# graphic-goose/ferreus_rbf_rs

Hardware: AMD Instinct MI355X
Metric: BBFMM matvecs/s (higher is better)
Workload: dtype f64; 1 GPU; 10000000 uniform 3D points, LinearRbf, order 7, 1 rhs, adaptive sparse tree, ACA eps=1e-7, set_weights + evaluate at the sources; points=10000000, kernel=LinearRbf, order=7, nrhs=1, parallelism=single GPU

## Files before the change

ferreus_rbf_rs_amd/_lib.py:

```python
from __future__ import annotations

import ctypes
import os

HERE = os.path.dirname(os.path.abspath(__file__))
LIB_PATH = os.environ.get("FERREUS_BBFMM_HIP_LIB") or os.path.join(HERE, "libferreus_bbfmm_hip.so")

OK, POINT_OUTSIDE_TREE, KERNEL_NO_GRADIENTS, BAD_ARGUMENT, DEVICE_ERROR, UNSUPPORTED, CALLBACK_FAILED = range(7)
FLAG_HOST_ONLY = 1
FLAG_M2L_SHARED_BASIS = 2
FLAG_DIRECT_SMALL_W_LEAVES = 4
FLAG_DETERMINISTIC = 8
N_PHASES = 11
PHASE_NAMES = ["gather", "P2M", "M2M", "M2L_stage1", "M2L_stage2", "P2L", "L2L", "P2P", "M2P",
               "L2P", "scatter"]

c_i32, c_i64, c_f64, c_u32 = ctypes.c_int32, ctypes.c_int64, ctypes.c_double, ctypes.c_uint32
c_p = ctypes.c_void_p


class Params(ctypes.Structure):
    _fields_ = [("max_points_per_cell", c_i64), ("compression_type", c_i32),
                ("epsilon", c_f64), ("eval_chunk_size", c_i64)]

# ... 67 lines not shown
    "bbfmm_isosurface_curvature_weight": (ctypes.c_int, [c_p, c_p, c_i32, c_p, c_p, c_p, c_p]),
    "bbfmm_isosurface_curvature_stats": (ctypes.c_int, [c_p, c_i32, c_p]),
    "bbfmm_isosurface_count": (c_i32, [c_p]),
    "bbfmm_isosurface_size": (ctypes.c_int, [c_p, c_i32, c_p, c_p]),
    "bbfmm_isosurface_copy": (ctypes.c_int, [c_p, c_i32, c_p, c_p]),
    "bbfmm_isosurface_error": (ctypes.c_char_p, [c_p]),
    "bbfmm_isosurface_destroy": (None, [c_p]),
    "bbfmm_prepare_target_subset": (ctypes.c_int, [c_p, c_p, c_i64]),
    "bbfmm_fast_matrix_vector_product": (ctypes.c_int, [c_p, c_p, c_i64, c_i64, c_p, c_i64, c_p,
                                                        c_i64, c_f64, c_p]),
    "bbfmm_matvec_device": (ctypes.c_int, [c_p, c_p, c_i64, c_i32, c_p, c_i64, c_i32]),
    "bbfmm_target_subset_create": (ctypes.c_int, [c_p, c_p, c_i64, c_p]),
    "bbfmm_matvec_subset_device": (ctypes.c_int, [c_p, c_i32, c_p, c_p, c_i32]),
    "bbfmm_stream": (c_p, [c_p]),
    "bbfmm_set_partition": (ctypes.c_int, [c_p, c_i32, c_i32]),
    "bbfmm_partition_row_count": (c_i64, [c_p]),
    "bbfmm_partition_rows": (ctypes.c_int, [c_p, c_p]),
    "bbfmm_partition_coarse_count": (c_i64, [c_p]),
    "bbfmm_matvec_partition_upward": (ctypes.c_int, [c_p, c_p, c_i64, c_i32, c_p, c_p]),
    "bbfmm_matvec_partition_finish": (ctypes.c_int, [c_p, c_p, c_p, c_i64, c_i32, c_p]),
    "bbfmm_partition_world": (c_i32, [c_p]),
    "bbfmm_partition_rank": (c_i32, [c_p]),
    "bbfmm_partition_bounds": (ctypes.c_int, [c_p, c_i32, c_p]),
    "bbfmm_matvec_partition_finish_sorted": (ctypes.c_int, [c_p, c_p, c_p, c_i64, c_p]),
    "bbfmm_partition_scatter": (ctypes.c_int, [c_p, c_p, c_i32, c_i32, c_i64, c_i32, c_p, c_i64]),
    "bbfmm_debug_partition_upward_counts": (ctypes.c_int, [c_p, c_p, c_p, c_p]),
    "bbfmm_debug_host_copy_rates": (ctypes.c_int, [c_i64, c_p]),
    "bbfmm_get_tree_stats": (ctypes.c_int, [c_p, c_p]),
    "bbfmm_tree_built_on_device": (ctypes.c_int, [c_p]),
    "bbfmm_last_evaluate_at_sources": (ctypes.c_int, [c_p]),
    "bbfmm_debug_targets_are_sources": (ctypes.c_int, [c_p, c_p, c_i64, c_i64]),
    "bbfmm_debug_rows_of_sources": (ctypes.c_int, [c_p, c_p, c_i64, c_i64, c_p]),
    "bbfmm_get_cells": (ctypes.c_int, [c_p, c_p, c_p]),
    "bbfmm_get_leaf_sources": (ctypes.c_int, [c_p, c_p, c_p]),
    "bbfmm_get_list": (ctypes.c_int, [c_p, ctypes.c_char, c_p, c_p, c_p]),
    "bbfmm_get_m2l_ranks": (ctypes.c_int, [c_p, c_p, c_p]),
    "bbfmm_get_m2l_operator": (ctypes.c_int, [c_p, c_i32, c_i32, c_p]),
    "bbfmm_get_m2l_factors": (ctypes.c_int, [c_p, c_i32, c_i32, c_p, c_p]),
    "bbfmm_get_permutation_tables": (ctypes.c_int, [c_p, c_p, c_p, c_p, c_p, c_p]),
    "bbfmm_points_to_leaves": (ctypes.c_int, [c_p, c_p, c_i64, c_i64, c_p, c_p]),
    "bbfmm_set_profiling": (ctypes.c_int, [c_p, c_i32]),
    "bbfmm_get_phase_ms": (ctypes.c_int, [c_p, c_p, c_p]),
    "bbfmm_reset_phase_ms": (ctypes.c_int, [c_p]),
    "bbfmm_mfma_f64_selftest": (ctypes.c_int, [c_p, c_p, c_p]),
    "bbfmm_fp64_valu_selftest": (ctypes.c_int, [c_p, c_p]),
    "bbfmm_debug_kernel_values": (ctypes.c_int, [c_i32, c_i32, ctypes.c_double, ctypes.c_double, c_p, c_i64, c_p, c_p, c_p]),
    "bbfmm_debug_math": (ctypes.c_int, [c_i32, c_i32, c_p, c_i64, c_p, c_p]),
    "bbfmm_debug_dense_m2m": (ctypes.c_int, [c_p, c_i32, c_p]),
    "bbfmm_debug_apply_m2l_tables_host": (ctypes.c_int, [c_p, c_p, c_p]),
    "bbfmm_debug_m2l_variants": (ctypes.c_int, [c_p, c_p, c_p]),
    "bbfmm_debug_m2l_pairs": (ctypes.c_int, [c_p, c_p, c_i64, c_p, c_p]),
    "bbfmm_debug_m2l_pairs_axes": (ctypes.c_int, [c_p, c_p, c_i64, c_p]),
    "bbfmm_debug_m2l_pairs_stage2": (ctypes.c_int, [c_p, c_p, c_i64, c_p, c_p]),
    "bbfmm_debug_m2l_s2_last_ksplit": (ctypes.c_int, [c_p, c_p]),
    "bbfmm_debug_get_coefficients": (ctypes.c_int, [c_p, ctypes.c_char, c_i32, c_p]),
    "bbfmm_debug_morton_encode": (ctypes.c_uint64, [c_i32, c_p, ctypes.c_uint64]),
    "bbfmm_debug_morton_decode": (None, [c_i32, ctypes.c_uint64, c_p, c_p]),
    "bbfmm_debug_morton_neighbours": (c_i32, [c_i32, ctypes.c_uint64, c_p]),
    "bbfmm_debug_direction_vectors": (c_i32, [c_i32, c_p]),
    "bbfmm_debug_reference_vectors": (ctypes.c_int, [c_p, c_p, c_p]),
    "bbfmm_givens_rotation": (None, [c_f64, c_f64, c_p, c_p, c_p]),
    "bbfmm_fgmres": (ctypes.c_int, [c_i64, c_p, c_p, c_p, c_p, c_p, c_p, c_i32, c_i32, c_i32, c_f64,
                                    c_p, c_p, c_p, c_p, c_p]),
    "bbfmm_schwarz_ddm_solver": (ctypes.c_int, [c_i64, c_p, c_p, c_p, c_p, c_p, c_i32, c_i32, c_f64,
                                                c_p, c_p, c_p, c_p, c_p]),
    "bbfmm_rbf_system_apply": (ctypes.c_int, [c_p, c_p, c_p, c_i64]),
    "bbfmm_ddm_params_defaults": (None, [c_p]),
    "bbfmm_ddm_params_for_points": (None, [c_i64, c_p]),
    "bbfmm_ddm_build": (ctypes.c_int, [c_p, c_i64, c_i32, c_i64, c_p, c_p]),
    "bbfmm_ddm_destroy": (None, [c_p]),
    "bbfmm_ddm_num_levels": (c_i32, [c_p]),
    "bbfmm_ddm_level_size": (c_i64, [c_p, c_i32]),
    "bbfmm_ddm_level_points": (ctypes.c_int, [c_p, c_i32, c_p]),
    "bbfmm_ddm_num_domains": (c_i64, [c_p, c_i32]),
    "bbfmm_ddm_domain_size": (c_i64, [c_p, c_i32, c_i64]),
    "bbfmm_ddm_domain": (ctypes.c_int, [c_p, c_i32, c_i64, c_p, c_p, c_p]),
    "bbfmm_schwarz_create": (ctypes.c_int, [c_p, c_p, c_i64, c_i32, c_i64, c_p, c_p, c_p]),
    "bbfmm_schwarz_create_sharded": (ctypes.c_int, [c_p, c_p, c_i64, c_i32, c_i64, c_p, c_p, c_i32, c_i32, c_p, c_i64, c_p, c_p, c_p]),
    "bbfmm_schwarz_factor_bytes": (c_i64, [c_p]),
    "bbfmm_schwarz_domains_owned": (c_i64, [c_p, c_i32, ctypes.POINTER(c_i64), ctypes.POINTER(c_i64)]),
    "bbfmm_schwarz_destroy": (None, [c_p]),
    "bbfmm_schwarz_basis_size": (c_i64, [c_p]),
    "bbfmm_schwarz_num_levels": (c_i32, [c_p]),
    "bbfmm_schwarz_monomial_matrix": (c_p, [c_p]),
    "bbfmm_debug_evaluate_monomials": (ctypes.c_int, [c_p, c_i64, c_i32, c_i64, c_i32, c_p, c_p, c_p]),
    "bbfmm_schwarz_apply": (ctypes.c_int, [c_p, c_p, c_p, c_i64]),
    "bbfmm_schwarz_level_size": (c_i64, [c_p, c_i32]),
    "bbfmm_schwarz_level_points": (ctypes.c_int, [c_p, c_i32, c_p]),
    "bbfmm_schwarz_debug_level_solve": (ctypes.c_int, [c_p, c_i32, c_p, c_p, c_i64, c_i32]),
    "bbfmm_ddm_debug_level_create": (ctypes.c_int, [c_p, c_i64, c_i32, c_i64, c_i64, c_p, c_p, c_p, c_p, c_i32, c_i32, c_p]),
    "bbfmm_ddm_debug_level_destroy": (None, [c_p]),
    "bbfmm_ddm_debug_level_info": (ctypes.c_int, [c_p, c_p]),
    "bbfmm_ddm_debug_level_layout": (ctypes.c_int, [c_p, c_p, c_p, c_p, c_p, c_p]),
    "bbfmm_ddm_debug_level_assembled": (ctypes.c_int, [c_p, c_p]),
    "bbfmm_ddm_debug_level_factor": (ctypes.c_int, [c_p, c_p]),
    "bbfmm_ddm_debug_level_solve": (ctypes.c_int, [c_p, c_p, c_p, c_i64, c_i32]),
    "bbfmm_schwarz_create_ex": (ctypes.c_int, [c_p, c_p, c_i64, c_i32, c_i64, c_p, c_i64, c_p, c_p, c_p]),
    "bbfmm_schwarz_create_sharded_ex": (ctypes.c_int, [c_p, c_p, c_i64, c_i32, c_i64, c_p, c_i64, c_p, c_p, c_i32, c_i32, c_p, c_i64,
                                                       c_p, c_p, c_p]),
    "bbfmm_ddm_debug_level_create_ex": (ctypes.c_int, [c_p, c_i64, c_i32, c_i64, c_p, c_i64, c_i64, c_p, c_p, c_p, c_p, c_i32, c_i32,
                                                       c_p]),
    "bbfmm_global_trend_transform": (ctypes.c_int, [c_i32, c_p, c_p, c_p, c_p]),
    "bbfmm_duplicate_cutoff_distance": (ctypes.c_int, [c_p, c_f64, c_p]),
    "bbfmm_remove_duplicates": (ctypes.c_int, [c_p, c_i64, c_i32, c_i64, c_f64, c_i32, c_p, c_p, c_p]),
    "bbfmm_debug_interpolant_terms": (ctypes.c_int, [c_i32, c_i32, c_p, c_p, c_i64, c_i64, c_p, c_i64, c_p, c_i64, c_p, c_i64]),
    "bbfmm_evaluate_interpolant": (ctypes.c_int, [c_p, c_i32, c_i32, c_p, c_i64, c_i32, c_i64, c_p, c_i64, c_i64, c_p, c_f64,
# ... 76 lines not shown
```

ferreus_rbf_rs_amd/csrc/capi.cpp:

```cpp
#include <cmath>
#include <cstddef>
#include <cstring>
#include <new>
#include <string>
#include <vector>

#include <algorithm>
#include <chrono>
#include <cstdlib>
#include <memory>

#include "device_group.hpp"
#include "ferreus_bbfmm_hip.h"
#include "fmm_tree.hpp"
#include "interpolant_terms.hpp"
#include "field_program.hpp"
#include "closure_triangulate.hpp"
#include "isosurface.hpp"
#include "isosurface_closure.hpp"
#include "isosurface_curvature.hpp"
#include "isosurface_intersect.hpp"
#include "morton.hpp"

struct bbfmm_handle {
// ... 1920 lines not shown
    if (d < 1 || d > 3 || !out) return -1;
    const int(*dirs)[3];
    const int n = bbfmm::direction_vectors(d, &dirs);
    for (int i = 0; i < n; ++i)
        for (int a = 0; a < d; ++a) out[i * d + a] = dirs[i][a];
    return n;
}
int bbfmm_debug_reference_vectors(const bbfmm_handle *h, int32_t *out, int32_t *n_ref_out) {
    if (!h) return BBFMM_BAD_ARGUMENT;
    const bbfmm::Operators &ops = h->tree.ops();
    if (n_ref_out) *n_ref_out = ops.n_ref;
    if (out) std::copy(ops.ref_vecs.begin(), ops.ref_vecs.end(), out);
    return BBFMM_OK;
}

int bbfmm_debug_m2l_variants(const bbfmm_handle *h, int64_t *n_variants, int64_t *n_cells) {
    if (!h) return BBFMM_BAD_ARGUMENT;
    int64_t nv = 0, nc = 0;
    h->tree.m2l_variant_stats(&nv, &nc);
    if (n_variants) *n_variants = nv;
    if (n_cells) *n_cells = nc;
    return BBFMM_OK;
}

int bbfmm_debug_m2l_pairs(const bbfmm_handle *h, int32_t *out, int64_t cap, int64_t *n_out, int32_t *pairs_on) {
    if (!h || !n_out) return BBFMM_BAD_ARGUMENT;
    std::vector<int32_t> v;
    h->tree.debug_m2l_pairs(&v);
    *n_out = static_cast<int64_t>(v.size());
    if (pairs_on) *pairs_on = h->tree.m2l_pairs() ? 1 : 0;
    if (out) std::copy(v.begin(), v.begin() + std::min<int64_t>(cap, *n_out), out);
    return BBFMM_OK;
}

int bbfmm_debug_m2l_pairs_axes(const bbfmm_handle *h, int32_t *out, int64_t cap, int64_t *n_out) {
    if (!h || !n_out) return BBFMM_BAD_ARGUMENT;
    std::vector<int32_t> v;
    h->tree.debug_m2l_pairs_axes(&v);
    *n_out = static_cast<int64_t>(v.size());
    if (out) std::copy(v.begin(), v.begin() + std::min<int64_t>(cap, *n_out), out);
    return BBFMM_OK;
}

int bbfmm_debug_m2l_pairs_stage2(const bbfmm_handle *h, int32_t *out, int64_t cap, int64_t *n_out, int32_t *pairs_on) {
    if (!h || !n_out) return BBFMM_BAD_ARGUMENT;
    std::vector<int32_t> v;
    h->tree.debug_m2l_pairs_stage2(&v);
    *n_out = static_cast<int64_t>(v.size());
    if (pairs_on) *pairs_on = h->tree.m2l_pairs_stage2() ? 1 : 0;
    if (out) std::copy(v.begin(), v.begin() + std::min<int64_t>(cap, *n_out), out);
    return BBFMM_OK;
}

int bbfmm_debug_m2l_s2_last_ksplit(const bbfmm_handle *h, int32_t *ksplit) {
    if (!h || !ksplit) return BBFMM_BAD_ARGUMENT;
    *ksplit = h->tree.debug_m2l_s2_last_ksplit();
    return BBFMM_OK;
}

int bbfmm_debug_get_coefficients(bbfmm_handle *h, char which, int32_t k, double *out) {
    GUARD(h) return h->tree.debug_get_coefficients(which, k, out);
    END_GUARD(h)
}

}

#include "ddm.hpp"
struct bbfmm_ddm {
    bbfmm::DdmTree tree;
};
extern "C" {
void bbfmm_ddm_params_defaults(bbfmm_ddm_params *out) {
    if (!out) return;
    const bbfmm::DdmParams p;
    out->leaf_threshold = p.leaf_threshold;
    out->overlap_quota = p.overlap_quota;
    out->coarse_ratio = p.coarse_ratio;
    out->coarse_threshold = p.coarse_threshold;
}

void bbfmm_ddm_params_for_points(int64_t n, bbfmm_ddm_params *out) {
    if (!out) return;
    bbfmm_ddm_params_defaults(out);
    out->coarse_threshold = std::max<int64_t>(out->coarse_threshold, n / 470 + 1);
}
int bbfmm_ddm_build(const double *points, int64_t n, int32_t d, int64_t ld, const bbfmm_ddm_params *params,
                    bbfmm_ddm **out) {
    if (!out) return BBFMM_BAD_ARGUMENT;
    *out = nullptr;
    bbfmm::DdmParams p;
    if (params) {
        p.leaf_threshold = params->leaf_threshold;
        p.overlap_quota = params->overlap_quota;
        p.coarse_ratio = params->coarse_ratio;
        p.coarse_threshold = params->coarse_threshold;
    }
    bbfmm_ddm *t = new (std::nothrow) bbfmm_ddm();
    if (!t) return BBFMM_DEVICE_ERROR;
    int rc = BBFMM_BAD_ARGUMENT;
    try {
        rc = bbfmm::build_ddm_tree(points, n, d, ld, p, &t->tree);
    } catch (...) {
        rc = BBFMM_DEVICE_ERROR;
    }
    if (rc != BBFMM_OK) {
        delete t;
// ... 43 lines not shown
```

ferreus_rbf_rs_amd/csrc/device.hpp:

```cpp
#pragma once
#include <hip/hip_runtime.h>

#include <cstdint>

#include "kernels.hpp"

namespace bbfmm {

constexpr int kMaxOrder = 16;
constexpr int kM2lTile = 128;
constexpr int kM2lS1Block = 176;
constexpr int kM2lS1BlockPairs = 160;
constexpr int kM2lSlotWindow = 128;
constexpr int kM2lBlkTwoDst = 1 << 30;

struct DevCheb {
    int p, d, n, n_pad;
    double polyn[kMaxOrder * kMaxOrder];
    double nodes[kMaxOrder];
    double xfer[2 * kMaxOrder * kMaxOrder];
};

struct ChebRef {
    const DevCheb *dev;
    int p, d, n, n_pad;
};

struct M2lClass {
    const double *vt_all;
    const int32_t *row_dst;
    const int32_t *row_dst2;
    const int32_t *blk_t0;
    int32_t yb0;
    int32_t n_rows;
    int32_t r_pad16;
    int32_t n_t;
    const double *u_all;
    int32_t k_pad;
    int32_t kp;
    const int32_t *cells;
    int32_t n_cells;
    const int32_t *cslot;
    const int64_t *cbase;
};

struct M2lTileDesc {
    int32_t level_class;
    int32_t first;
    int32_t count;
    int32_t q_first;
    int32_t q_count;
    int32_t pad;
};

void launch_gather_weights(const double *w, int64_t ldw, int K, const int32_t *order, int64_t N,
                           double *w_sorted, hipStream_t s);
void launch_gather_weights_subset(const double *w, int64_t ldw, int K, const int32_t *order, const int32_t *pos, int64_t n_pos,
                                  int64_t N, double *w_sorted, hipStream_t s);
constexpr int kMaxScatterParts = 64;
struct ScatterParts {
    int n;
    int64_t bound[kMaxScatterParts + 1];
};
void launch_scatter_parts(const double *all, const ScatterParts &parts, int64_t m_max, int K, const int32_t *order, double *out,
                          int64_t ldo, hipStream_t s);
void launch_sum_slots(const double *slots, int n_slots, int64_t len, double *out, hipStream_t s);
void launch_scatter_output(const double *out_sorted, int64_t n, int K, const int32_t *perm,
                           double *out, int64_t ldo, int accumulate, hipStream_t s);
void launch_gather_rows(const double *src, int64_t ld_src, int ncols, const int32_t *idx, int64_t n,
                        double *dst, int64_t ld_dst, hipStream_t s);

void launch_p2m(const ChebRef &ch, const double *const *src_xyz, const double *w_sorted, int64_t N,
                int K, int64_t C, const int32_t *leaf_cells, int n_leaves, const int32_t *pt_begin,
                const int32_t *pt_end, const double *centers, const double *lengths, double *M,
                hipStream_t s);
int launch_m2m(const ChebRef &ch, int K, int64_t C, const int32_t *parents, int n_parents,
               const int64_t *child_ptr, const int32_t *child_idx, const int32_t *octant, double *M,
               hipStream_t s);
int launch_l2l(const ChebRef &ch, int K, int64_t C, const int32_t *cells, int n_cells,
               const int32_t *parent, const int32_t *octant, const uint8_t *active, double *L,
               hipStream_t s);

void launch_m2l_stage1(const M2lClass *classes, const M2lTileDesc *tiles, const int32_t *tile_idx, int n_tiles,
                       int n_pad, int max_slot_t, int K, int64_t C, const double *M, double *cbuf,
                       int64_t cbuf_len, hipStream_t s, bool own_blocks = false, int max_blocks = 8, int ne16 = 0, int s_ee = 0,
                       int s_eo = 0);
void launch_m2l_parity(const double *M, int n_pad, double *Mp, int n_par, int ne16, int n_e, int n_o, int p, int64_t rows,
                       hipStream_t s);
struct M2lParityOffsets {
    int32_t v[4];
};
void launch_m2l_parity2(const double *M, int n_pad, double *Mp, int n_par, M2lParityOffsets off, int p, int p2, int64_t rows,
                        hipStream_t s);
void launch_m2l_stage2(const M2lClass *classes, const M2lTileDesc *tiles, const int32_t *tile_idx, int n_tiles,
                       int n_pad, int K, int64_t C, const double *cbuf, int64_t cbuf_len,
                       const uint16_t *qlist, double *L, hipStream_t s, bool allow_ksplit = true);
struct M2lS2PairsPlan {
    int ga, gb, ce, co;
    int ne16() const { return 16 * ga * ce; }
    int n_par() const { return 16 * (ga * ce + gb * co); }
};
M2lS2PairsPlan m2l_s2_pairs_plan(int groups_even, int groups_odd);
bool launch_m2l_stage2_pairs(const M2lClass *classes, const M2lTileDesc *tiles, const int32_t *tile_idx, int n_tiles,
                             const M2lS2PairsPlan &plan, int K, int64_t C, const double *cbuf, int64_t cbuf_len,
                             const uint16_t *qlist, double *Lp, hipStream_t s, bool allow_ksplit = true, int *ksplit_out = nullptr);
void launch_m2l_unparity(const double *Lp, int n_par, int ne16, double *L, int n, int n_pad, int n_e, int n_o, int p, int64_t rows,
                         hipStream_t s);
void launch_m2l_zero_segments(const int32_t *segs, int64_t n_segs, int K, double *cbuf, int64_t cbuf_len, hipStream_t s);
void launch_m2l_basis(const M2lClass *classes, const M2lTileDesc *tiles, int n_tiles, int in_ld, int out_ld, int K,
                      int64_t C, const double *in, double *out, hipStream_t s);
void launch_small_gemm(bool trans_a, int M, int N, int Kd, const double *A, int64_t lda, const double *B, int64_t ldb,
                       double *Cm, int64_t ldc, hipStream_t s);

struct M2lAssembleTv {
    int32_t perm;
    int32_t rank;
    int32_t row;
    int64_t vt_off;
    int64_t u_off;
};
struct M2lAssembleClass {
    const M2lAssembleTv *src, *tgt;
    int32_t n_src, n_tgt, r_pad16, k_pad, max_rank;
    int32_t n_e, n_o, ne16, n_par, p;
    int32_t u_npar, u_ne16, u_rows, u_ne, u_no;
    int32_t s1_axes;
    M2lParityOffsets s1_off;
};
void launch_m2l_assemble(const M2lAssembleClass &c, int n, int n_pad, bool compressed, const double *ops,
                         const int32_t *invperm, double *vt_all, double *u_all, hipStream_t s);

struct DirectJobs {
    int n_jobs;
    const int32_t *job_cell;
    const int32_t *tgt_begin, *tgt_end;
    const int64_t *run_ptr;
    const int32_t *runs;
};
void launch_p2p(const KernelSpec &ks, int d, const DirectJobs &jobs, const double *const *tgt_xyz,
                int64_t n_tgt, const double *const *src_xyz, const double *w_sorted, int64_t N, int K,
                double *out_sorted, double *grad_sorted, hipStream_t s, bool fixed_plan = false);
constexpr int kSymMaxRhs = 4;
void launch_p2p_sym(const KernelSpec &ks, int n_jobs, const int32_t *tgt_begin, const int32_t *tgt_end,
                    const int64_t *run_range, int n_leaf_jobs, const int32_t *l_tgt_begin, const int32_t *l_tgt_end,
                    const int64_t *l_run_range, int n_wave_jobs, const int32_t *w_tgt_begin, const int32_t *w_tgt_end,
                    const int64_t *w_run_range, const int32_t *runs3, int32_t tgt_off, const double *const *src_xyz,
                    const double *w_sorted, int64_t ldw, int K, double *out_sorted, int64_t ldo, hipStream_t s);
int p2p_sym_rows_per_job();
int p2p_sym3_rows_per_job();
int p2p_sym_wave_rows();
int64_t p2p_sym_wave_min_jobs();
int wx_sym_rows_per_job();
int wx_sym3_rows_per_job();
void launch_wx_sym(const KernelSpec &ks, const ChebRef &ch, int n_jobs, const int32_t *tgt_begin, const int32_t *tgt_end,
                   const int64_t *w_range, int n_leaf_jobs, const int32_t *l_tgt_begin, const int32_t *l_tgt_end,
                   const int64_t *l_w_range, const int32_t *w_cells, const double *centers, const double *lengths,
                   const double *const *src_xyz, const double *w_sorted, int64_t ldw, int K, const double *M, double *L,
                   int64_t ld_ml, double *out_sorted, int64_t ldo, int out_off, int out_n, hipStream_t s);
void launch_m2p(const KernelSpec &ks, const ChebRef &ch, int n_jobs, const int32_t *tgt_begin,
                const int32_t *tgt_end, const int64_t *w_begin, const int64_t *w_end,
                const int32_t *w_cells,
                const double *centers, const double *lengths, const double *const *tgt_xyz,
                int64_t n_tgt, int K, int64_t C, const double *M, double *out_sorted,
                double *grad_sorted, hipStream_t s, bool fixed_plan = false);
void launch_p2l(const KernelSpec &ks, const ChebRef &ch, int n_jobs, const int32_t *cells,
                const int64_t *run_ptr, const int32_t *runs, const double *centers,
                const double *lengths, const double *const *src_xyz, const double *w_sorted,
                int64_t N, int K, int64_t C, double *L, hipStream_t s);
void launch_l2p(const ChebRef &ch, int n_jobs, const int32_t *leaf_cells, const int32_t *tgt_begin,
                const int32_t *tgt_end, const double *centers, const double *lengths,
                const double *const *tgt_xyz, int64_t n_tgt, int K, int64_t C, const double *L,
                double *out_sorted, double *grad_sorted, hipStream_t s);

bool l2p_order_supported(int p, int d);

int mfma_f64_selftest(double *tflops, int *layout_errors, double *info);
int valu_f64_selftest(double *tflops, double *mhz);
int debug_kernel_values_device(const KernelSpec &ks, const double *r2, int64_t n, double *value, double *value_g, double *factor);
int debug_math_device(int which, const double *x, int64_t n, double *out, double *out2);

// ... 2 lines not shown
```

ferreus_rbf_rs_amd/csrc/device_m2l.hip:

```cpp
#include "device_common.hpp"

#include <cmath>

namespace bbfmm {

typedef __attribute__((address_space(3))) void *lptr_t;

__device__ inline unsigned lds_offset(const double *p) {
    return static_cast<unsigned>(reinterpret_cast<uintptr_t>((lptr_t)p));
}
__device__ inline unsigned uniform_u32(unsigned v) { return __builtin_amdgcn_readfirstlane(v); }
__device__ inline const double *uniform_ptr(const double *p) {
    const uintptr_t v = reinterpret_cast<uintptr_t>(p);
    const unsigned lo = __builtin_amdgcn_readfirstlane(static_cast<unsigned>(v));
    const unsigned hi = __builtin_amdgcn_readfirstlane(static_cast<unsigned>(v >> 32));
    return reinterpret_cast<const double *>((static_cast<uintptr_t>(hi) << 32) | lo);
}
__device__ inline void dma16(const double *g, unsigned lds_wave_byte_offset) {
    asm volatile("s_mov_b32 m0, %1\n\ts_nop 0\n\tglobal_load_lds_dwordx4 %0, off" ::"v"(g),
                 "s"(uniform_u32(lds_wave_byte_offset))
                 : "memory");
}
__device__ inline void dma4(const int32_t *g, unsigned lds_wave_byte_offset) {
    asm volatile("s_mov_b32 m0, %1\n\ts_nop 0\n\tglobal_load_lds_dword %0, off" ::"v"(g),
// ... 392 lines not shown
    const int zmax = n_tiles * 8 < n_cu ? std::max(8, std::min(max_blocks, 32)) : 8;
    int zsplit = 1;
    double best = 1e300;
    for (int z = 1; z <= zmax; ++z) {
        const double rounds = std::ceil(static_cast<double>(n_tiles) * z / n_cu);
        const double cost = rounds / z * (1.0 + 0.005 * z);
        if (cost < best - 1e-12) {
            best = cost;
            zsplit = z;
        }
    }
    const int n_colblocks = own_blocks ? 1 : zsplit;
    if (ne16 > 0) {
        const int64_t packed = static_cast<int64_t>(ne16) | (static_cast<int64_t>(s_ee & 0xffff) << 32) | (static_cast<int64_t>(s_eo & 0x7fff) << 48);
        m2l_gemm_launch<kM2lS1BlockPairs / 16, 1, 1, true>(classes, tiles, n_tiles, n_pad, 0, n_colblocks, K, C, M, packed, cbuf, cbuf_len,
                                                      nullptr, slot_t, tile_idx, s);
        return;
    }
    m2l_dispatch_chunks<1>(kM2lS1Block / 16, classes, tiles, n_tiles, n_pad, n_colblocks, K, C, M, 0, cbuf, cbuf_len, nullptr,
                           slot_t, tile_idx, s);
}

static int m2l_s2_ksplit(int64_t wgs, bool allow_ksplit) {
    static const int ks_env = [] {
        const int v = env_int("BBFMM_M2L_S2_KSPLIT", 0);
        return v >= 1 && v <= 32 ? v : 0;
    }();
    if (!allow_ksplit) return 1;
    if (ks_env > 0) return ks_env;
    const int n_cu = device_cu_count();
    int ksplit = 1;
    if (wgs * 2 <= static_cast<int64_t>(kM2lS2KsplitFill) * n_cu) {
        double best = 1e300;
        for (int ks = 1; ks <= 16; ++ks) {
            const double cost = std::ceil(static_cast<double>(wgs * ks) / n_cu) * (0.05 + 1.0 / ks);
            if (cost < best - 1e-12) {
                best = cost;
                ksplit = ks;
            }
        }
    }
    return ksplit;
}

void launch_m2l_stage2(const M2lClass *classes, const M2lTileDesc *tiles, const int32_t *tile_idx, int n_tiles,
                       int n_pad, int K, int64_t C, const double *cbuf, int64_t cbuf_len, const uint16_t *qlist,
                       double *L, hipStream_t s, bool allow_ksplit) {
    if (n_tiles == 0) return;
    static const int z = env_int("BBFMM_M2L_S2_ZSPLIT", 2) == 1 ? 1 : 2;
    const int ksplit = m2l_s2_ksplit(static_cast<int64_t>(n_tiles) * z * K, allow_ksplit);
    m2l_dispatch_chunks<2>(n_pad / 16, classes, tiles, n_tiles, n_pad, z, K, C, cbuf, cbuf_len, L, 0, qlist, ksplit > 1 ? ksplit : 0, tile_idx, s);
}

template <int NG16>
__device__ __forceinline__ void m2l_s2_pairs_body(const M2lClass &cls, const M2lTileDesc &tile, int n_par, int g16, bool odd,
                                                  int zk, int ksplit, int64_t C, const double *__restrict__ in, int64_t in_len,
                                                  double *__restrict__ out, const uint16_t *__restrict__ qlist,
                                                  const int32_t *__restrict__ tile_idx, double *lds) {
    const int kr = blockIdx.y;
    const int tid = threadIdx.x, wave = tid >> 6, lane = tid & 63;
    const int ld = n_par;
    const int q_lo = tile.q_count * zk / ksplit;
    const int nq = tile.q_count * (zk + 1) / ksplit - q_lo;
    const uint16_t *ql = qlist + tile.q_first + q_lo;
    const int kp = cls.kp, kp16 = kp >> 4;
    const double *opbase = cls.u_all + 16 * g16;

    constexpr int OP_CHUNKS = 2 * NG16;
    constexpr int NCH = (OP_CHUNKS + 7) / 8;
    constexpr int OP_DOUBLES = OP_CHUNKS * 128;
    constexpr int BUF = OP_DOUBLES + 4096;
    constexpr int NP = NG16 / 2, NS = NG16 & 1;
    unsigned voff[NCH];
#pragma unroll
    for (int i = 0; i < NCH; ++i) {
        const int c = wave + 8 * i;
        if (c < 4 * NP) {
            const int e = c / (NP > 0 ? NP : 1), pr = c - e * NP, k = lane >> 4, p = lane & 15;
            voff[i] = (unsigned)(((4 * k + e) * ld + 32 * pr + 2 * p) * 8);
        } else {
            const int e = 2 * (c - 4 * NP) + (lane >> 5), r = lane & 31, k = r >> 3, pair = r & 7;
            voff[i] = (unsigned)(((4 * k + e) * ld + 32 * NP + 2 * pair) * 8);
        }
    }
    auto cell_p = [&](int pos) {
        const int q = pos < tile.count ? pos : 0;
        return tile.pad ? tile_idx[tile.first + q] : tile.first + q;
    };
    const double *cptr[2];
#pragma unroll
    for (int h = 0; h < 2; ++h) {
        const int tg = 2 * h + (lane >> 5), eh = (lane >> 4) & 1, k = (lane >> 2) & 3, j = lane & 3;
        const int p = cell_p(wave * 16 + 4 * tg + j);
        cptr[h] = in + (int64_t)kr * in_len + cls.cbase[p] + 4 * k + 2 * eh;
    }
    const unsigned lds0 = lds_offset(lds);
    const int64_t qstride = (int64_t)16 * ld;
    auto stage = [&](int qi, int buf) {
        const int q = (int)uniform_u32(ql[qi]);
#pragma unroll
        for (int i = 0; i < NCH; ++i)
            if (wave + 8 * i < OP_CHUNKS)
                dma16s(opbase + q * qstride, voff[i], lds0 + (unsigned)(buf * BUF + (wave + 8 * i) * 128) * 8u);
#pragma unroll
        for (int h = 0; h < 2; ++h)
            dma16(cptr[h] + kp + 16 * q, lds0 + (unsigned)(buf * BUF + OP_DOUBLES + 2048 + (2 * wave + h) * 128) * 8u);
        if (q < kp16) {
#pragma unroll
            for (int h = 0; h < 2; ++h)
                dma16(cptr[h] + 16 * q, lds0 + (unsigned)(buf * BUF + OP_DOUBLES + (2 * wave + h) * 128) * 8u);
        }
        return q < kp16;
    };

    double acc[4][NG16];
#pragma unroll
    for (int tg = 0; tg < 4; ++tg)
#pragma unroll
        for (int g = 0; g < NG16; ++g) acc[tg][g] = 0.0;

    const int bk = lane >> 4, bj = lane & 3;
    const bool wave_live = wave * 16 < tile.count;
    const int di = lane >> 4, db = (lane >> 2) & 3, dj = lane & 3;
    const double sgn = odd ? -1.0 : 1.0;
    bool pair_cur = false;
    if (nq > 0) pair_cur = stage(0, 0);
    wait_dma_and_barrier();
    for (int sidx = 0; sidx < nq; ++sidx) {
        const double *op = lds + (sidx & 1) * BUF + lane;
        const double2 *op2 = reinterpret_cast<const double2 *>(lds + (sidx & 1) * BUF) + lane;
        const double *cx = lds + (sidx & 1) * BUF + OP_DOUBLES + wave * 256 + (bk * 4 + bj) * 2;
        bool pair_next = false;
        if (sidx + 1 < nq) pair_next = stage(sidx + 1, (sidx + 1) & 1);
        if (wave_live) {
            double bq[4][4];
#pragma unroll
            for (int tg = 0; tg < 4; ++tg)
#pragma unroll
                for (int eh = 0; eh < 2; ++eh) {
                    const double2 y = *reinterpret_cast<const double2 *>(cx + 2048 + ((tg * 2 + eh) * 16) * 2);
                    bq[tg][2 * eh] = y.x;
                    bq[tg][2 * eh + 1] = y.y;
                }
            if (pair_cur) {
#pragma unroll
                for (int tg = 0; tg < 4; ++tg)
#pragma unroll
                    for (int eh = 0; eh < 2; ++eh) {
                        const double2 x = *reinterpret_cast<const double2 *>(cx + ((tg * 2 + eh) * 16) * 2);
                        bq[tg][2 * eh] = x.x + sgn * bq[tg][2 * eh];
                        bq[tg][2 * eh + 1] = x.y + sgn * bq[tg][2 * eh + 1];
                    }
            }
#pragma unroll
            for (int e = 0; e < 4; ++e) {
#pragma unroll
                for (int pr = 0; pr < NP; ++pr) {
                    const double2 a = op2[(e * NP + pr) * 64];
#pragma unroll
                    for (int tg = 0; tg < 4; ++tg) {
                        acc[tg][2 * pr] = __builtin_amdgcn_mfma_f64_4x4x4f64(a.x, bq[tg][e], acc[tg][2 * pr], 0, 0, 0);
                        acc[tg][2 * pr + 1] = __builtin_amdgcn_mfma_f64_4x4x4f64(a.y, bq[tg][e], acc[tg][2 * pr + 1], 0, 0, 0);
                    }
                }
                if (NS) {
                    const double a = op[4 * NP * 128 + e * 64];
#pragma unroll
                    for (int tg = 0; tg < 4; ++tg)
                        acc[tg][NG16 - 1] = __builtin_amdgcn_mfma_f64_4x4x4f64(a, bq[tg][e], acc[tg][NG16 - 1], 0, 0, 0);
                }
            }
        }
        pair_cur = pair_next;
        wait_dma_and_barrier();
    }
    const int col0 = 16 * g16;
#pragma unroll
    for (int tg = 0; tg < 4; ++tg) {
        const int tp = wave * 16 + 4 * tg + dj;
        if (tp < tile.count) {
            const int cell = cls.cells[cell_p(tp)];
            double *Lc = out + ((int64_t)kr * C + cell) * n_par + col0;
            if (ksplit > 1) {
#pragma unroll
                for (int pr = 0; pr < NP; ++pr) {
                    unsafeAtomicAdd(Lc + 32 * pr + 2 * (4 * db + di), acc[tg][2 * pr]);
                    unsafeAtomicAdd(Lc + 32 * pr + 2 * (4 * db + di) + 1, acc[tg][2 * pr + 1]);
                }
                if (NS) unsafeAtomicAdd(Lc + 32 * NP + 4 * db + di, acc[tg][NG16 - 1]);
            } else {
#pragma unroll
                for (int pr = 0; pr < NP; ++pr)
                    *reinterpret_cast<double2 *>(Lc + 32 * pr + 2 * (4 * db + di)) = make_double2(acc[tg][2 * pr], acc[tg][2 * pr + 1]);
                if (NS) Lc[32 * NP + 4 * db + di] = acc[tg][NG16 - 1];
            }
        }
    }
}

template <int GA, int GB>
__global__ __launch_bounds__(512, 1) void m2l_s2_pairs_kernel(const M2lClass *__restrict__ classes, const M2lTileDesc *__restrict__ tiles,
                                                              int n_par, int ce, int co, int ksplit, int64_t C,
                                                              const double *__restrict__ in, int64_t in_len, double *__restrict__ out,
                                                              const uint16_t *__restrict__ qlist, const int32_t *__restrict__ tile_idx) {
    extern __shared__ double lds[];
    const M2lTileDesc tile = tiles[blockIdx.x];
    const M2lClass cls = classes[tile.level_class];
    const int zcols = ce + co;
    const int zk = (int)blockIdx.z / zcols, zc = (int)blockIdx.z - zk * zcols;
    if (zc < ce) m2l_s2_pairs_body<GA>(cls, tile, n_par, zc * GA, false, zk, ksplit, C, in, in_len, out, qlist, tile_idx, lds);
    else m2l_s2_pairs_body<GB>(cls, tile, n_par, ce * GA + (zc - ce) * GB, true, zk, ksplit, C, in, in_len, out, qlist, tile_idx, lds);
}

#define M2L_S2_PAIR_WIDTHS(X) X(13, 10) X(13, 11) X(8, 8) X(7, 7) X(5, 4) X(4, 4) X(2, 2) X(1, 1)
#define M2L_S2_WIDTH_ENTRY(A, B) {A, B},
static constexpr int kM2lS2PairWidths[][2] = {M2L_S2_PAIR_WIDTHS(M2L_S2_WIDTH_ENTRY)};
#undef M2L_S2_WIDTH_ENTRY

M2lS2PairsPlan m2l_s2_pairs_plan(int groups_even, int groups_odd) {
    M2lS2PairsPlan best{1, 1, std::max(groups_even, 1), std::max(groups_odd, 1)};
    int best_cost = 1 << 30;
    for (const auto &w : kM2lS2PairWidths) {
        const int ce = std::max(1, (groups_even + w[0] - 1) / w[0]), co = std::max(1, (groups_odd + w[1] - 1) / w[1]);
        const int cost = ce * (w[0] + 2) + co * (w[1] + 2);
        if (cost < best_cost) {
            best_cost = cost;
            best = M2lS2PairsPlan{w[0], w[1], ce, co};
        }
    }
    return best;
}

template <int GA, int GB>
static void m2l_s2_pairs_launch(const M2lClass *classes, const M2lTileDesc *tiles, const int32_t *tile_idx, int n_tiles,
                                const M2lS2PairsPlan &plan, int ksplit, int K, int64_t C, const double *cbuf, int64_t cbuf_len,
                                const uint16_t *qlist, double *Lp, hipStream_t s) {
    const size_t lds = 2 * sizeof(double) * (size_t)(2 * (GA > GB ? GA : GB) * 128 + 4096);
    static std::atomic<uint64_t> attr_set[4] = {{0}, {0}, {0}, {0}};
    (void)allow_large_dynamic_lds(reinterpret_cast<const void *>(&m2l_s2_pairs_kernel<GA, GB>), lds, attr_set);
    hipLaunchKernelGGL((m2l_s2_pairs_kernel<GA, GB>), dim3(n_tiles, K, (plan.ce + plan.co) * ksplit), dim3(512), lds, s, classes, tiles,
                       plan.n_par(), plan.ce, plan.co, ksplit, C, cbuf, cbuf_len, Lp, qlist, tile_idx);
}

bool launch_m2l_stage2_pairs(const M2lClass *classes, const M2lTileDesc *tiles, const int32_t *tile_idx, int n_tiles,
                             const M2lS2PairsPlan &plan, int K, int64_t C, const double *cbuf, int64_t cbuf_len,
                             const uint16_t *qlist, double *Lp, hipStream_t s, bool allow_ksplit, int *ksplit_out) {
    if (n_tiles == 0) return true;
    const int ksplit = m2l_s2_ksplit(static_cast<int64_t>(n_tiles) * (plan.ce + plan.co) * K, allow_ksplit);
    if (ksplit_out) *ksplit_out = ksplit;
#define M2L_S2_DISPATCH(A, B)                                                                                            \
    if (plan.ga == A && plan.gb == B) {                                                                                  \
        m2l_s2_pairs_launch<A, B>(classes, tiles, tile_idx, n_tiles, plan, ksplit, K, C, cbuf, cbuf_len, qlist, Lp, s);  \
        return true;                                                                                                     \
    }
    M2L_S2_PAIR_WIDTHS(M2L_S2_DISPATCH)
#undef M2L_S2_DISPATCH
    return false;
}

__global__ __launch_bounds__(256) void m2l_unparity_kernel(const double *__restrict__ Lp, int n_par, int ne16, double *__restrict__ L,
                                                           int n, int n_pad, int n_e, int n_o, int p, int p1, int64_t rows) {
    const int64_t row = static_cast<int64_t>(blockIdx.x) * 4 + (threadIdx.x >> 6);
    if (row >= rows) return;
    const double *src = Lp + row * n_par;
    double *dst = L + row * n_pad;
    for (int j = threadIdx.x & 63; j < n_e; j += 64) {
        const double e = src[j];
        if (j < n_o) {
            const double o = src[ne16 + j];
            dst[j] = e + o;
            dst[j + (p - 1 - 2 * (j / p1)) * p1] = e - o;
        } else {
            dst[j] = e;
        }
    }
    for (int j = n + (threadIdx.x & 63); j < n_pad; j += 64) dst[j] = 0.0;
}

void launch_m2l_unparity(const double *Lp, int n_par, int ne16, double *L, int n, int n_pad, int n_e, int n_o, int p, int64_t rows,
                         hipStream_t s) {
    if (rows <= 0) return;
    const int p1 = n_e / ((p + 1) / 2);
    hipLaunchKernelGGL(m2l_unparity_kernel, dim3(static_cast<unsigned>((rows + 3) / 4)), dim3(256), 0, s, Lp, n_par, ne16, L, n, n_pad, n_e,
                       n_o, p, p1, rows);
}

__global__ __launch_bounds__(256) void m2l_parity_kernel(const double *__restrict__ M, int n_pad, double *__restrict__ Mp, int n_par,
                                                         int ne16, int n_e, int n_o, int p, int p1, int64_t rows) {
    const int64_t row = static_cast<int64_t>(blockIdx.x) * 4 + (threadIdx.x >> 6);
    if (row >= rows) return;
    const double *src = M + row * n_pad;
    double *dst = Mp + row * n_par;
    for (int j = threadIdx.x & 63; j < n_e; j += 64) {
        const double v = src[j];
        if (j < n_o) {
            const double w = src[j + (p - 1 - 2 * (j / p1)) * p1];
            dst[j] = v + w;
            dst[ne16 + j] = v - w;
        } else {
            dst[j] = v;
        }
    }
}

void launch_m2l_parity(const double *M, int n_pad, double *Mp, int n_par, int ne16, int n_e, int n_o, int p, int64_t rows,
                       hipStream_t s) {
    if (rows <= 0) return;
    const int p1 = n_e / ((p + 1) / 2);
    hipLaunchKernelGGL(m2l_parity_kernel, dim3(static_cast<unsigned>((rows + 3) / 4)), dim3(256), 0, s, M, n_pad, Mp, n_par, ne16, n_e,
                       n_o, p, p1, rows);
}

__global__ __launch_bounds__(256) void m2l_parity2_kernel(const double *__restrict__ M, int n_pad, double *__restrict__ Mp, int n_par,
                                                          M2lParityOffsets off, int p, int p2, int64_t rows) {
    const int64_t row = static_cast<int64_t>(blockIdx.x) * 4 + (threadIdx.x >> 6);
    if (row >= rows) return;
    const double *src = M + row * n_pad;
    double *dst = Mp + row * n_par;
    const int h = (p + 1) / 2, f = p / 2;
    for (int e = threadIdx.x & 63; e < h * h * p2; e += 64) {
        const int i0 = e / (h * p2), i1 = (e - i0 * h * p2) / p2, r = e - (i0 * h + i1) * p2;
        const int m = (i0 * p + i1) * p2 + r;
        const int dx = (p - 1 - 2 * i0) * p * p2, dy = (p - 1 - 2 * i1) * p2;
        const bool cx = i0 >= f, cy = i1 >= f;
        const double v = src[m], vx = src[m + dx], vy = src[m + dy], vxy = src[m + dx + dy];
        const double e0 = cx ? v : v + vx, e1 = cx ? vy : vy + vxy, o0 = v - vx, o1 = vy - vxy;
        const int je = (i0 * h + i1) * p2 + r, jo = (i0 * f + i1) * p2 + r;
        dst[off.v[0] + je] = cy ? e0 : e0 + e1;
        if (!cy) dst[off.v[1] + jo] = e0 - e1;
        if (!cx) dst[off.v[2] + je] = cy ? o0 : o0 + o1;
        if (!cx && !cy) dst[off.v[3] + jo] = o0 - o1;
    }
}

void launch_m2l_parity2(const double *M, int n_pad, double *Mp, int n_par, M2lParityOffsets off, int p, int p2, int64_t rows,
                        hipStream_t s) {
    if (rows <= 0) return;
// ... 127 lines not shown
    const bool cx = i0 >= f, cy = i1 >= f;
    const int32_t *inv = invperm + static_cast<int64_t>(tv.perm) * n;
    const double *s0 = ops + tv.vt_off + static_cast<int64_t>(inv[m]) * tv.rank;
    const double *sx = ops + tv.vt_off + static_cast<int64_t>(inv[m + dx]) * tv.rank;
    const double *sy = ops + tv.vt_off + static_cast<int64_t>(inv[m + dy]) * tv.rank;
    const double *sxy = ops + tv.vt_off + static_cast<int64_t>(inv[m + dx + dy]) * tv.rank;
    const int je = (i0 * h + i1) * p2 + r, jo = (i0 * f + i1) * p2 + r;
    double *dee = vt_all + static_cast<int64_t>(c.s1_off.v[0] + je) * c.r_pad16 + tv.row;
    double *deo = vt_all + static_cast<int64_t>(c.s1_off.v[1] + jo) * c.r_pad16 + tv.row;
    double *doe = vt_all + static_cast<int64_t>(c.s1_off.v[2] + je) * c.r_pad16 + tv.row;
    double *doo = vt_all + static_cast<int64_t>(c.s1_off.v[3] + jo) * c.r_pad16 + tv.row;
    const double wx = cx ? 1.0 : 0.5, wy = cy ? 1.0 : 0.5;
    for (int kk = 0; kk < tv.rank; ++kk) {
        const double v = s0[kk], vx = sx[kk], vy = sy[kk], vxy = sxy[kk];
        const double e0 = cx ? v : v + vx, e1 = cx ? vy : vy + vxy, o0 = v - vx, o1 = vy - vxy;
        dee[kk] = wx * wy * (cy ? e0 : e0 + e1);
        if (!cy) deo[kk] = wx * wy * (e0 - e1);
        if (!cx) doe[kk] = wx * wy * (cy ? o0 : o0 + o1);
        if (!cx && !cy) doo[kk] = wx * wy * (o0 - o1);
    }
}

__global__ __launch_bounds__(256) void assemble_u_kernel(M2lAssembleClass c, int n, int n_pad, const double *__restrict__ ops,
                                                         const int32_t *__restrict__ invperm, double *__restrict__ u_all) {
    const int pos = blockIdx.y;
    const M2lAssembleTv tv = c.tgt[pos];
    const int64_t t = static_cast<int64_t>(blockIdx.x) * 256 + threadIdx.x;
    if (t >= static_cast<int64_t>(tv.rank) * n) return;
    const int kk = static_cast<int>(t / n), i = static_cast<int>(t % n);
    u_all[static_cast<int64_t>(tv.row + kk) * n_pad + i] = ops[tv.u_off + static_cast<int64_t>(kk) * n + invperm[static_cast<int64_t>(tv.perm) * n + i]];
}

__global__ __launch_bounds__(256) void assemble_u_parity_kernel(M2lAssembleClass c, int n, const double *__restrict__ ops,
                                                                const int32_t *__restrict__ invperm, double *__restrict__ u_all) {
    const M2lAssembleTv tv = c.tgt[blockIdx.y];
    const int64_t t = static_cast<int64_t>(blockIdx.x) * 256 + threadIdx.x;
    if (t >= static_cast<int64_t>(tv.rank) * c.u_ne) return;
    const int kk = static_cast<int>(t / c.u_ne), i = static_cast<int>(t % c.u_ne);
    const int p1 = n / c.p;
    const int ri = i + (c.p - 1 - 2 * (i / p1)) * p1;
    const int32_t *inv = invperm + static_cast<int64_t>(tv.perm) * n;
    const double *ucol = ops + tv.u_off + static_cast<int64_t>(kk) * n;
    double *dst = u_all + static_cast<int64_t>(tv.row + kk) * c.u_npar;
    const double a = ucol[inv[i]];
    if (i >= c.u_no) {
        dst[i] = a;
    } else {
        const double b = ucol[inv[ri]];
        dst[i] = 0.5 * (a + b);
        dst[c.u_ne16 + i] = 0.5 * (a - b);
    }
}

void launch_m2l_assemble(const M2lAssembleClass &c, int n, int n_pad, bool compressed, const double *ops,
                         const int32_t *invperm, double *vt_all, double *u_all, hipStream_t s) {
    (void)hipMemsetAsync(vt_all, 0, static_cast<size_t>(c.n_e > 0 ? c.n_par : n_pad) * c.r_pad16 * sizeof(double), s);
    (void)hipMemsetAsync(u_all, 0, (c.u_npar > 0 ? static_cast<size_t>(c.u_rows) * c.u_npar : static_cast<size_t>(c.k_pad) * n_pad) * sizeof(double), s);
    if (c.n_src > 0 && c.n_e > 0 && c.s1_axes == 2) {
        const int h = (c.p + 1) / 2, n_ee = h * h * (n / (c.p * c.p));
        hipLaunchKernelGGL(assemble_vt_parity2_kernel, dim3(static_cast<unsigned>((static_cast<int64_t>(c.n_src) * n_ee + 255) / 256)), dim3(256),
                           0, s, c, n, ops, invperm, vt_all);
    } else if (c.n_src > 0 && c.n_e > 0)
        hipLaunchKernelGGL(assemble_vt_parity_kernel, dim3(static_cast<unsigned>((static_cast<int64_t>(c.n_src) * c.n_e + 255) / 256)), dim3(256),
                           0, s, c, n, ops, invperm, vt_all);
    else if (c.n_src > 0)
        hipLaunchKernelGGL(assemble_vt_kernel, dim3(static_cast<unsigned>((static_cast<int64_t>(c.n_src) * n + 255) / 256)), dim3(256), 0, s, c, n, n_pad,
                           compressed ? 1 : 0, ops, invperm, vt_all);
    if (c.n_tgt > 0 && c.max_rank > 0 && c.u_npar > 0)
        hipLaunchKernelGGL(assemble_u_parity_kernel, dim3(static_cast<unsigned>((static_cast<int64_t>(c.max_rank) * c.u_ne + 255) / 256), c.n_tgt),
                           dim3(256), 0, s, c, n, ops, invperm, u_all);
    else if (c.n_tgt > 0 && c.max_rank > 0)
        hipLaunchKernelGGL(assemble_u_kernel, dim3(static_cast<unsigned>((static_cast<int64_t>(c.max_rank) * n + 255) / 256), c.n_tgt), dim3(256), 0, s, c,
                           n, n_pad, ops, invperm, u_all);
}

}
```

ferreus_rbf_rs_amd/csrc/fmm_m2l_tables.cpp:

```cpp
#include "fmm_tree_impl.hpp"

namespace bbfmm {

void FmmTree::fill_m2l_operator_arrays(const HostM2lClass &hc, std::vector<double> *vt_all,
                                       std::vector<double> *u_all) const {
    const int n_pad = round_up(ops_.n, 32);
    vt_all->resize(static_cast<size_t>(m2l_pairs_ ? m2l_npar_ : n_pad) * hc.r_pad16);
    u_all->resize(m2l_pairs2_ ? static_cast<size_t>(hc.k_pad - hc.kp) * m2l_s2_plan_.n_par() : static_cast<size_t>(hc.k_pad) * n_pad);
    fill_m2l_operator_arrays(hc, vt_all->data(), u_all->data());
}

void FmmTree::fill_m2l_operator_arrays(const HostM2lClass &hc, double *vt_all, double *u_all) const {
    const int n = ops_.n, n_pad = round_up(n, 32);
    const bool compressed = ops_.compression != kCompressionNone;
    const auto &lops = ops_.m2l[hc.level];
    auto zero = [](double *p, size_t len) {
        parallel_for_chunks(static_cast<int64_t>(len), int64_t(1) << 18, [&](int64_t b, int64_t e) {
            std::memset(p + b, 0, static_cast<size_t>(e - b) * sizeof(double));
        });
    };
    zero(vt_all, static_cast<size_t>(m2l_pairs_ ? m2l_npar_ : n_pad) * hc.r_pad16);
    zero(u_all, m2l_pairs2_ ? static_cast<size_t>(hc.k_pad - hc.kp) * m2l_s2_plan_.n_par() : static_cast<size_t>(hc.k_pad) * n_pad);
    struct RowSrc {
        const M2lOperator *op;
// ... 21 lines not shown
                for (int kk = 0; kk < r; ++kk) {
                    double v = 0.0;
                    for (int g = 0; g < 4; ++g)
                        if (nd[g] >= 0) v += sg[g] * rs.op->vt[static_cast<size_t>(rs.inv[nd[g]]) * r + kk];
                    dst[rs.first_row + kk] = w * v;
                }
            }
        });
    } else if (m2l_pairs_) {
        parallel_for(m2l_ne_, 8, [&](int64_t j) {
            const bool centre = j >= m2l_no_;
            const int rj = m2l_rho(static_cast<int>(j));
            double *de = vt_all + static_cast<size_t>(j) * hc.r_pad16;
            double *dod = vt_all + static_cast<size_t>(m2l_ne16_ + j) * hc.r_pad16;
            for (const RowSrc &rs : row_src) {
                const int r = rs.op->rank;
                const double *s0 = &rs.op->vt[static_cast<size_t>(rs.inv[j]) * r], *s1 = &rs.op->vt[static_cast<size_t>(rs.inv[rj]) * r];
                for (int kk = 0; kk < r; ++kk) {
                    if (centre) {
                        de[rs.first_row + kk] = s0[kk];
                    } else {
                        de[rs.first_row + kk] = 0.5 * (s0[kk] + s1[kk]);
                        dod[rs.first_row + kk] = 0.5 * (s0[kk] - s1[kk]);
                    }
                }
            }
        });
    } else {
        parallel_for(n, 8, [&](int64_t m) {
            double *dst = vt_all + static_cast<size_t>(m) * hc.r_pad16;
            for (const RowSrc &rs : row_src) {
                const int r = rs.op->rank;
                const int im = rs.inv[m];
                if (compressed) {
                    const double *src = &rs.op->vt[static_cast<size_t>(im) * r];
                    for (int kk = 0; kk < r; ++kk) dst[rs.first_row + kk] = src[kk];
                } else {
                    dst[rs.first_row + im] = 1.0;
                }
            }
        });
    }
    if (m2l_pairs2_) {
        const int n_par = m2l_s2_plan_.n_par(), ne16 = m2l_s2_plan_.ne16();
        parallel_for(static_cast<int64_t>(hc.tgt_tv.size()), 1, [&](int64_t pos) {
            if (hc.tgt_pair[pos] == -2) return;
            const int tv = hc.tgt_tv[pos];
            const M2lOperator &op = lops[ops_.ref_lookup[tv]];
            const int32_t *inv = &ops_.invperm[static_cast<size_t>(ops_.perm_lookup[tv]) * n];
            const int row0 = hc.tgt_off[pos] - (hc.tgt_pair[pos] >= 0 ? 0 : hc.kp);
            for (int kk = 0; kk < op.rank; ++kk) {
                double *dst = u_all + static_cast<size_t>(row0 + kk) * n_par;
                const double *ucol = &op.u[static_cast<size_t>(kk) * n];
                for (int i = 0; i < m2l_ne_; ++i) {
                    const double a = ucol[inv[i]], b = ucol[inv[m2l_rho(i)]];
                    if (i >= m2l_no_) {
                        dst[i] = a;
                    } else {
                        dst[i] = 0.5 * (a + b);
                        dst[ne16 + i] = 0.5 * (a - b);
                    }
                }
            }
        });
        return;
    }
    parallel_for(static_cast<int64_t>(hc.tgt_tv.size()), 1, [&](int64_t pos) {
        const int tv = hc.tgt_tv[pos];
        const M2lOperator &op = lops[ops_.ref_lookup[tv]];
        const int32_t *inv = &ops_.invperm[static_cast<size_t>(ops_.perm_lookup[tv]) * n];
        for (int kk = 0; kk < op.rank; ++kk) {
            double *dst = u_all + static_cast<size_t>(hc.tgt_off[pos] + kk) * n_pad;
            const double *ucol = &op.u[static_cast<size_t>(kk) * n];
            for (int i = 0; i < n; ++i) dst[i] = ucol[inv[i]];
        }
    });
}

int FmmTree::build_m2l_tables() {
    const HostTree &t = tree_;
    const int d = d_, n = ops_.n;
    const int ncls = 1 << d, nvec = ops_.n_vec;
    const bool compressed = ops_.compression != kCompressionNone;
    m2l_host_.clear();
    m2l_variants_.clear();
    m2l_tiles1_h_.clear();
    m2l_tile_idx1_h_.clear();
    m2l_classes_h_.clear();
    m2l_tiles_h_.clear();
    m2l_qlist_h_.clear();
    m2l_batches_.clear();
    m2l_batch_of_class_.clear();
    m2l_group_ops_.clear();
    cbuf_batch_len_ = 0;
    cbuf_total_len_ = 0;
    m2l_flops_k1_ = 0;
    m2l_flops_level_.clear();
    if (t.depth < 2) return BBFMM_OK;
    if (!host_only_) {
        size_t free_b = 0, total_b = 0;
        if (hipMemGetInfo(&free_b, &total_b) == hipSuccess && total_b > 0)
            m2l_budget_bytes_ = std::max<int64_t>(int64_t(4) << 30, static_cast<int64_t>(total_b / 16));
    }
    if (const char *e = std::getenv("BBFMM_M2L_CBUF_MB")) {
        const double mb = std::atof(e);
        if (mb > 0) m2l_budget_bytes_ = static_cast<int64_t>(mb * 1048576.0);
    }

    auto comp = [&](int tv, int a) { return ops_.all_vecs[static_cast<size_t>(tv) * d + a]; };
    {
        const char *e = std::getenv("BBFMM_M2L_S1_PAIRS");
        m2l_pairs_ = !(e && std::atoi(e) == 0) && compressed && !shared_basis_ && d >= 2 && ops_.p >= 2;
        const char *e2 = std::getenv("BBFMM_M2L_S2_PAIRS");
        m2l_pairs2_ = !(e2 && std::atoi(e2) == 0) && compressed && !shared_basis_ && d >= 2 && ops_.p >= 2;
        m2l_partner_.assign(static_cast<size_t>(nvec), -1);
        m2l_s1_block_ = m2l_pairs_ ? kM2lS1BlockPairs : kM2lS1Block;
        const int p1 = n / ops_.p;
        m2l_ne_ = (ops_.p + 1) / 2 * p1;
        m2l_no_ = ops_.p / 2 * p1;
        m2l_ne16_ = round_up(m2l_ne_, 16);
        m2l_npar_ = m2l_ne16_ + round_up(m2l_no_, 16);
        m2l_s2_plan_ = m2l_s2_pairs_plan(m2l_ne16_ / 16, round_up(m2l_no_, 16) / 16);
        for (int tv = 0; tv < nvec && (m2l_pairs_ || m2l_pairs2_); ++tv) {
            if (comp(tv, 0) == 0) continue;
            int rt = -1;
            for (int u = 0; u < nvec && rt < 0; ++u) {
                bool same = comp(u, 0) == -comp(tv, 0);
                for (int a = 1; a < d; ++a) same = same && comp(u, a) == comp(tv, a);
                if (same) rt = u;
            }
            if (rt < 0 || ops_.ref_lookup[rt] != ops_.ref_lookup[tv]) continue;
            const int32_t *it = &ops_.invperm[static_cast<size_t>(ops_.perm_lookup[tv]) * n];
            const int32_t *ir = &ops_.invperm[static_cast<size_t>(ops_.perm_lookup[rt]) * n];
            bool ok = true;
            for (int m = 0; m < n && ok; ++m) ok = ir[m] == it[m2l_rho(m)];
            if (ok) m2l_partner_[static_cast<size_t>(tv)] = rt;
        }
        m2l_partner_y_.assign(static_cast<size_t>(nvec), -1);
        for (int tv = 0; tv < nvec && m2l_pairs_; ++tv) {
            if (comp(tv, 1) == 0) continue;
            int rt = -1;
            for (int u = 0; u < nvec && rt < 0; ++u) {
                bool same = comp(u, 1) == -comp(tv, 1);
                for (int a = 0; a < d; ++a) same = same && (a == 1 || comp(u, a) == comp(tv, a));
                if (same) rt = u;
            }
            if (rt < 0 || ops_.ref_lookup[rt] != ops_.ref_lookup[tv]) continue;
            const int32_t *it = &ops_.invperm[static_cast<size_t>(ops_.perm_lookup[tv]) * n];
            const int32_t *ir = &ops_.invperm[static_cast<size_t>(ops_.perm_lookup[rt]) * n];
            bool ok = true;
            for (int m = 0; m < n && ok; ++m) ok = ir[m] == it[m2l_rho_y(m)];
            if (ok) m2l_partner_y_[static_cast<size_t>(tv)] = rt;
        }
    }
    auto far = [&](int tv) {
        int mx = 0;
        for (int a = 0; a < d; ++a) mx = std::max(mx, std::abs(comp(tv, a)));
        return mx >= 2;
    };
    std::vector<std::vector<int>> tgt_list(ncls), src_list(ncls), tpos_tgt(ncls, std::vector<int>(nvec, -1)),
        tpos_src(ncls, std::vector<int>(nvec, -1));
    for (int o = 0; o < ncls; ++o)
        for (int tv = 0; tv < nvec; ++tv) {
            if (!far(tv)) continue;
            bool okt = true, oks = true;
            for (int a = 0; a < d; ++a) {
                const int oa = (o >> a) & 1, ta = comp(tv, a);
                okt = okt && ta >= oa - 3 && ta <= oa + 2;
                oks = oks && ta >= -2 - oa && ta <= 3 - oa;
            }
            if (okt) {
                tpos_tgt[o][tv] = static_cast<int>(tgt_list[o].size());
                tgt_list[o].push_back(tv);
            }
            if (oks) {
                tpos_src[o][tv] = static_cast<int>(src_list[o].size());
                src_list[o].push_back(tv);
            }
        }
    auto pairs_first = [&](std::vector<int> *list, std::vector<int> *tpos) {
        std::vector<int> ordered, singles;
        std::vector<uint8_t> used(static_cast<size_t>(nvec), 0);
        for (int tv : *list) {
            const int rt = m2l_partner_[static_cast<size_t>(tv)];
            if (used[static_cast<size_t>(tv)]) continue;
            if (rt >= 0 && (*tpos)[rt] >= 0 && m2l_partner_[static_cast<size_t>(rt)] == tv) {
                const int first = comp(tv, 0) > 0 ? tv : rt;
                ordered.push_back(first);
                ordered.push_back(first == tv ? rt : tv);
                used[static_cast<size_t>(tv)] = used[static_cast<size_t>(rt)] = 1;
            } else {
                singles.push_back(tv);
// ... 97 lines not shown
        for (int i = 1; i < 4; ++i) off2.v[i] = off2.v[i - 1] + round_up(len[i - 1], 16);
        const int npar2 = off2.v[3] + round_up(len[3], 16);
        std::vector<std::vector<int>> src_xy = src_list;
        for (int o = 0; o < ncls; ++o) order_axes(&src_xy[o], nullptr);
        for (int level = 2; level <= t.depth; ++level) {
            std::vector<uint8_t> has(static_cast<size_t>(ncls), 0);
            for (int64_t c = t.level_ptr[level]; c < t.level_ptr[level + 1]; ++c) has[t.octant[c]] = 1;
            for (int o = 0; o < ncls; ++o) {
                if (!has[static_cast<size_t>(o)]) continue;
                std::vector<int32_t> marks;
                const int rows1 = mark_pairs_at(level, 1, src_list[o], &marks, nullptr, nullptr, nullptr, nullptr);
                const int rows2 = mark_pairs_at(level, 2, src_xy[o], &marks, nullptr, nullptr, nullptr, nullptr);
                m2l_work_[0] += static_cast<int64_t>(round_up(std::max(rows1, 1), m2l_s1_block_) / m2l_s1_block_) * (m2l_npar_ / 16);
                m2l_work_[1] += static_cast<int64_t>(round_up(std::max(rows2, 1), m2l_s1_block_) / m2l_s1_block_) * (npar2 / 16);
            }
        }
        const char *e = std::getenv("BBFMM_M2L_S1_AXES");
        const int want = e ? std::atoi(e) : 0;
        if (want == 2 || (want != 1 && m2l_work_[1] < m2l_work_[0])) {
            m2l_axes_ = 2;
            m2l_s1_off_ = off2;
            m2l_ne16_ = off2.v[2];
            m2l_npar_ = npar2;
            m2l_s_ee_ = off2.v[1] / 16;
            m2l_s_eo_ = (off2.v[2] - off2.v[1]) / 16;
            for (int o = 0; o < ncls; ++o) {
                src_list[o] = src_xy[o];
                for (size_t i = 0; i < src_list[o].size(); ++i) tpos_src[o][src_list[o][i]] = static_cast<int>(i);
            }
            m2l_par_node_.assign(static_cast<size_t>(npar2) * 4, -1);
            m2l_par_sign_.assign(static_cast<size_t>(npar2) * 4, 0);
            for (int i0 = 0; i0 < h; ++i0)
                for (int i1 = 0; i1 < h; ++i1)
                    for (int r = 0; r < p2; ++r) {
                        const int m = (i0 * p + i1) * p2 + r;
                        const bool cx = i0 >= f, cy = i1 >= f;
                        const int nodes[4] = {m, m2l_rho(m), m2l_rho_y(m), m2l_rho_y(m2l_rho(m))};
                        const int je = (i0 * h + i1) * p2 + r, jo = (i0 * f + i1) * p2 + r;
                        for (int part = 0; part < 4; ++part) {
                            const bool ox = part >= 2, oy = part & 1;
                            if ((ox && cx) || (oy && cy)) continue;
                            const size_t k = static_cast<size_t>(off2.v[part] + (oy ? jo : je));
                            for (int g = 0; g < 4; ++g) {
                                const bool gx = g & 1, gy = g & 2;
                                if ((gx && cx) || (gy && cy)) continue;
                                m2l_par_node_[4 * k + g] = nodes[g];
                                m2l_par_sign_[4 * k + g] = static_cast<int8_t>(((gx && ox) != (gy && oy)) ? -1 : 1);
                            }
                        }
                    }
        }
    }
    std::vector<std::vector<int32_t>> tgt_pair(ncls);
    for (int o = 0; o < ncls; ++o) {
        const std::vector<int> &tl = tgt_list[o];
        tgt_pair[o].assign(tl.size(), -1);
        for (size_t pos = 0; m2l_pairs2_ && pos + 1 < tl.size(); ++pos)
            if (m2l_partner_[static_cast<size_t>(tl[pos])] == tl[pos + 1] && m2l_partner_[static_cast<size_t>(tl[pos + 1])] == tl[pos]) {
                tgt_pair[o][pos] = static_cast<int32_t>(pos + 1);
                tgt_pair[o][pos + 1] = -2;
                ++pos;
            }
    }
    auto target_class = [&](int o, int tv) {
        int oc = 0;
        for (int a = 0; a < d; ++a) {
            const int v = ((o >> a) & 1) + comp(tv, a);
            oc |= (((v % 2) + 2) % 2) << a;
        }
        return oc;
    };

    std::vector<int32_t> pos_in_class(t.n_cells(), -1);
    int64_t bad_pairs = 0;
    auto slot_layout = [&](int level, std::vector<std::vector<int>> *off_tgt, std::vector<int> *k_pad, std::vector<int> *kp_out = nullptr) {
        const auto &lops = ops_.m2l[level];
        off_tgt->assign(ncls, {});
        k_pad->assign(ncls, 0);
        if (kp_out) kp_out->assign(ncls, 0);
        for (int o = 0; o < ncls; ++o) {
            int lead = 0;
            for (size_t pos = 0; pos < tgt_list[o].size(); ++pos)
                if (tgt_pair[o][pos] >= 0) lead += round_up(lops[ops_.ref_lookup[tgt_list[o][pos]]].rank, 2);
            const int kp = round_up(lead, 16);
            int off = 0, off_s = 2 * kp;
            for (size_t pos = 0; pos < tgt_list[o].size(); ++pos) {
                const int seg = round_up(lops[ops_.ref_lookup[tgt_list[o][pos]]].rank, 2);
                if (tgt_pair[o][pos] >= 0) {
                    (*off_tgt)[o].push_back(off);
                } else if (tgt_pair[o][pos] == -2) {
                    (*off_tgt)[o].push_back(kp + off);
                    off += seg;
                } else {
                    (*off_tgt)[o].push_back(off_s);
                    off_s += seg;
                }
            }
            (*k_pad)[o] = round_up(std::max(off_s, 16), 16);
            if (kp_out) (*kp_out)[o] = kp;
        }
    };
    std::vector<int> level_groups(static_cast<size_t>(t.depth) + 1, 1);
    std::vector<std::vector<int>> batch_of(static_cast<size_t>(t.depth) + 1, std::vector<int>(ncls, -1));
    {
        const int64_t budget = std::max<int64_t>(m2l_budget_bytes_ / 8 - 128, 1);
        std::vector<std::vector<int64_t>> class_len(static_cast<size_t>(t.depth) + 1, std::vector<int64_t>(ncls, 0));
        for (int level = 2; level <= t.depth; ++level) {
            std::vector<std::vector<int>> off_tgt;
            std::vector<int> k_pad;
            slot_layout(level, &off_tgt, &k_pad);
            for (int64_t c = t.level_ptr[level]; c < t.level_ptr[level + 1]; ++c) class_len[level][t.octant[c]] += k_pad[t.octant[c]];
        }
        int64_t cur_len = 0;
        for (int level = 2; level <= t.depth; ++level) {
            int64_t len = 0;
            for (int64_t v : class_len[level]) len += v;
            cbuf_total_len_ += len;
            int G = 1;
            if (len > budget)
                for (G = 2; G < ncls; G *= 2) {
                    int64_t worst = 0;
                    for (int g = 0; g < G; ++g) {
                        int64_t gl = 0;
                        for (int o = g * ncls / G; o < (g + 1) * ncls / G; ++o) gl += class_len[level][o];
                        worst = std::max(worst, gl);
                    }
                    if (worst <= budget) break;
                }
            if (G >= ncls) {
                G = ncls;
                int64_t worst = 0;
                for (int64_t v : class_len[level]) worst = std::max(worst, v);
                if (worst > budget && std::getenv("BBFMM_VERBOSE"))
                    std::fprintf(stderr, "[bbfmm] warning: level %d needs %.1f MB of M2L intermediate per right-hand side even "
                                         "with one batch per target class; the budget of %.1f MB (BBFMM_M2L_CBUF_MB) is exceeded\n",
                                 level, worst * 8.0 / 1048576.0, m2l_budget_bytes_ / 1048576.0);
            }
            level_groups[level] = G;
            if (G == 1 && !m2l_batches_.empty() && m2l_batches_.back().groups == 1 && cur_len + len <= budget) {
                m2l_batches_.back().level_hi = level;
                cur_len += len;
                for (int o = 0; o < ncls; ++o) batch_of[level][o] = static_cast<int>(m2l_batches_.size()) - 1;
                continue;
            }
            for (int g = 0; g < G; ++g) {
                M2lBatch b;
                b.level_lo = b.level_hi = level;
                b.groups = G;
                b.group = g;
                for (int o = g * ncls / G; o < (g + 1) * ncls / G; ++o) batch_of[level][o] = static_cast<int>(m2l_batches_.size());
                m2l_batches_.push_back(b);
            }
            cur_len = len;
        }
    }
    std::vector<std::vector<M2lTileDesc>> tiles1_of_batch(m2l_batches_.size());
    std::vector<int32_t> variant_batch;
    std::vector<std::vector<int32_t>> zero_of_batch(m2l_batches_.size());
    for (int level = 2; level <= t.depth; ++level) {
        const auto &lops = ops_.m2l[level];
        auto rank_of = [&](int tv) { return lops[ops_.ref_lookup[tv]].rank; };
        std::vector<std::vector<int>> off_tgt;
        std::vector<int> k_pad, kp_cls;
        slot_layout(level, &off_tgt, &k_pad, &kp_cls);
        const size_t first_class = m2l_host_.size();
        auto mark_pairs = [&](const std::vector<int> &tvs, std::vector<int32_t> *src_pair) {
            return mark_pairs_at(level, m2l_axes_, tvs, src_pair, nullptr, nullptr, nullptr, nullptr);
        };
        auto stage1_rows = [&](int o, const std::vector<int> &tvs, HostM2lClass *hcp) {
            HostM2lClass &hc = *hcp;
            hc.n_t = static_cast<int>(tvs.size());
            std::vector<int32_t> first_row;
            hc.n_rows = mark_pairs_at(level, m2l_axes_, tvs, &hc.src_pair, &first_row, &hc.src_kind, &hc.yb0, &hc.pad_cols);
            hc.r_pad16 = round_up(std::max(hc.n_rows, 1), m2l_s1_block_);
            if (hc.yb0 < 0) hc.yb0 = hc.r_pad16 / m2l_s1_block_;
            hc.row_tpos.assign(hc.r_pad16, -1);
            hc.row_off.assign(hc.r_pad16, 0);
            hc.row_tpos2.assign(hc.r_pad16, -1);
            hc.row_off2.assign(hc.r_pad16, 0);
            hc.src_tv = tvs;
            int row = 0;
            hc.src_row0.assign(tvs.size(), 0);
            hc.src_row1.assign(tvs.size(), 0);
            for (size_t pos = 0; pos < tvs.size(); ++pos) {
                if (hc.src_pair[pos] == -2) {
                    hc.src_row0[pos] = hc.src_row0[pos - 1];
                    hc.src_row1[pos] = hc.src_row1[pos - 1];
                    continue;
                }
                const int tv = tvs[pos];
                const int oc = target_class(o, tv);
                const int base_off = off_tgt[oc][tpos_tgt[oc][tv]];
                int base_off2 = 0;
                if (hc.src_pair[pos] >= 0) {
                    const int tv2 = tvs[pos + 1], oc2 = target_class(o, tv2);
                    base_off2 = off_tgt[oc2][tpos_tgt[oc2][tv2]];
                }
                if (rank_of(tv) > 0) row = first_row[pos];
                hc.src_row0[pos] = row;
                for (int kk = 0; kk < rank_of(tv); ++kk, ++row) {
                    hc.row_tpos[row] = static_cast<int32_t>(pos);
                    hc.row_off[row] = base_off + kk;
                    if (hc.src_pair[pos] >= 0) {
                        hc.row_tpos2[row] = static_cast<int32_t>(pos + 1);
                        hc.row_off2[row] = base_off2 + kk;
                    }
                }
                hc.src_row1[pos] = row;
                row = round_up(row, 2);
            }
            const int n_blk = hc.r_pad16 / m2l_s1_block_;
            m2l_max_blocks_ = std::max(m2l_max_blocks_, n_blk);
            hc.blk_t0.assign(n_blk, 0);
            hc.row_dst.assign(hc.r_pad16, -1);
            hc.row_dst2.assign(hc.r_pad16, -1);
            for (int b = 0; b < n_blk; ++b) {
                int t0 = -1, t1 = -1;
                bool two = false;
                for (int r = b * m2l_s1_block_; r < (b + 1) * m2l_s1_block_; ++r) {
                    if (hc.row_tpos[r] < 0) continue;
                    if (t0 < 0) t0 = hc.row_tpos[r];
                    t1 = std::max(hc.row_tpos[r], hc.row_tpos2[r]);
                    two = two || hc.row_tpos2[r] >= 0;
                }
                if (t0 < 0) continue;
                hc.blk_t0[b] = t0 | (two ? kM2lBlkTwoDst : 0);
                m2l_slot_t_ = std::max(m2l_slot_t_, t1 - t0 + 1);
                for (int r = b * m2l_s1_block_; r < (b + 1) * m2l_s1_block_; ++r) {
                    if (hc.row_tpos[r] < 0) continue;
                    if (hc.row_off[r] >= (1 << 24) || hc.row_off2[r] >= (1 << 24)) return false;
                    hc.row_dst[r] = ((hc.row_tpos[r] - t0) << 24) | hc.row_off[r];
                    if (hc.row_tpos2[r] >= 0) hc.row_dst2[r] = ((hc.row_tpos2[r] - t0) << 24) | hc.row_off2[r];
                }
            }
            return true;
        };
        m2l_host_.resize(first_class + ncls);
        m2l_group_ops_.resize(first_class + ncls);
        for (int64_t c = t.level_ptr[level]; c < t.level_ptr[level + 1]; ++c)
            m2l_host_[first_class + t.octant[c]].cells.push_back(static_cast<int32_t>(c));
        {
            std::vector<uint64_t> key(static_cast<size_t>(t.level_ptr[level + 1] - t.level_ptr[level]));
            const int64_t c_lo = t.level_ptr[level];
            for (int64_t c = c_lo; c < t.level_ptr[level + 1]; ++c) {
                uint64_t hsh = 1469598103934665603ull;
                const int64_t nv = t.v.ptr[c + 1] - t.v.ptr[c];
                uint64_t bits[6] = {0, 0, 0, 0, 0, 0};
                for (int64_t q = t.v.ptr[c]; q < t.v.ptr[c + 1]; ++q) {
                    const int tv = t.v_tidx[q];
                    if (tv >= 0 && tv < 384) bits[tv >> 6] |= 1ull << (tv & 63);
                }
                for (uint64_t b : bits) hsh = (hsh ^ b) * 1099511628211ull;
                key[static_cast<size_t>(c - c_lo)] = (static_cast<uint64_t>(1023 - std::min<int64_t>(nv, 1023)) << 54) | (hsh >> 10);
            }
            parallel_for(ncls, 1, [&](int64_t o) {
                auto &cells = m2l_host_[first_class + static_cast<size_t>(o)].cells;
                std::stable_sort(cells.begin(), cells.end(), [&](int32_t a, int32_t b) {
                    return key[static_cast<size_t>(a - c_lo)] < key[static_cast<size_t>(b - c_lo)];
                });
                for (size_t i = 0; i < cells.size(); ++i) pos_in_class[cells[i]] = static_cast<int32_t>(i);
            });
        }
        for (int o = 0; o < ncls; ++o) {
            HostM2lClass &hc = m2l_host_[first_class + o];
            hc.level = level;
            hc.octant = o;
            hc.n_t = static_cast<int>(src_list[o].size());
            hc.k_pad = k_pad[o];
            hc.kp = kp_cls[o];
            hc.tgt_pair = tgt_pair[o];
            if (!stage1_rows(o, src_list[o], &hc)) return fail(BBFMM_BAD_ARGUMENT, "M2L slot too long for the packed row table");
            if (hc.cells.empty()) continue;
            hc.tgt_tv = tgt_list[o];
            hc.tgt_off = off_tgt[o];
            if (host_only_) fill_m2l_operator_arrays(hc, &hc.vt_all, &hc.u_all);
            hc.cbase.resize(hc.cells.size());
            int64_t &cursor = m2l_batches_[static_cast<size_t>(batch_of[level][o])].len;
            for (size_t i = 0; i < hc.cells.size(); ++i) {
                hc.cbase[i] = cursor;
                cursor += hc.k_pad;
            }
            hc.cslot.resize(hc.cells.size() * static_cast<size_t>(hc.n_t));
            {
                int32_t *cs = hc.cslot.data();
                parallel_for_chunks(static_cast<int64_t>(hc.cslot.size()), int64_t(1) << 18, [&](int64_t b, int64_t e) {
                    std::fill(cs + b, cs + e, int32_t(-1));
                });
            }
        }
        {
            const int64_t b0 = t.level_ptr[level], nb_cells = t.level_ptr[level + 1] - b0;
            constexpr int64_t kChunkB = 2048;
            const int64_t nch = (nb_cells + kChunkB - 1) / kChunkB;
            std::vector<double> flops_part(static_cast<size_t>(std::max<int64_t>(nch, 1)), 0.0);
            std::vector<int64_t> bad_part(static_cast<size_t>(std::max<int64_t>(nch, 1)), 0);
            parallel_for_chunks(nb_cells, kChunkB, [&](int64_t lo, int64_t hi) {
                double fl = 0.0;
                int64_t bad = 0;
                for (int64_t B = b0 + lo; B < b0 + hi; ++B) {
                    const HostM2lClass &hb = m2l_host_[first_class + t.octant[B]];
                    const int64_t base = hb.cbase[pos_in_class[B]];
                    for (int64_t q = t.v.ptr[B]; q < t.v.ptr[B + 1]; ++q) {
                        const int32_t V = t.v.idx[q];
                        const int tv = t.v_tidx[q];
                        HostM2lClass &hv = m2l_host_[first_class + t.octant[V]];
                        const int ps = (tv >= 0 && tv < nvec) ? tpos_src[t.octant[V]][tv] : -1;
                        if (ps < 0 || t.level[V] != level || tpos_tgt[t.octant[B]][tv] < 0) {
                            ++bad;
                            continue;
                        }
                        hv.cslot[static_cast<size_t>(pos_in_class[V]) * hv.n_t + ps] = static_cast<int32_t>(base / 2);
                        const int r = rank_of(tv);
                        fl += compressed ? 4.0 * n * r : 2.0 * n * static_cast<double>(n);
                    }
                }
                flops_part[static_cast<size_t>(lo / kChunkB)] = fl;
                bad_part[static_cast<size_t>(lo / kChunkB)] = bad;
            });
            double level_flops = 0.0;
            for (double f : flops_part) level_flops += f;
            m2l_flops_k1_ += level_flops;
            if (m2l_flops_level_.size() <= static_cast<size_t>(level)) m2l_flops_level_.resize(static_cast<size_t>(level) + 1, 0.0);
            m2l_flops_level_[static_cast<size_t>(level)] = level_flops;
// ... 521 lines not shown
                          cbuf.begin() + 2 * (static_cast<int64_t>(m2l_zero_h_[static_cast<size_t>(2 * z)]) + m2l_zero_h_[static_cast<size_t>(2 * z + 1)]), 0.0);
        for (int32_t ti = mb.t1_first; ti < mb.t1_first + mb.t1_count; ++ti) {
            const M2lTileDesc &td = m2l_tiles1_h_[static_cast<size_t>(ti)];
            const bool variant = static_cast<size_t>(td.level_class) >= m2l_host_.size();
            const HostM2lClass &hc = variant ? m2l_variants_[static_cast<size_t>(td.level_class) - m2l_host_.size()]
                                             : m2l_host_[static_cast<size_t>(td.level_class)];
            if (hc.vt_all.empty()) return BBFMM_UNSUPPORTED;
            if (m2l_batch_of_class_[static_cast<size_t>(td.level_class)] != static_cast<int32_t>(b)) return BBFMM_BAD_ARGUMENT;
            for (int32_t q = 0; q < td.count; ++q) {
                const size_t pos = static_cast<size_t>(td.pad ? m2l_tile_idx1_h_[static_cast<size_t>(td.first + q)] : td.first + q);
                ++seen[hc.cells[pos]];
                const double *Mv = M + static_cast<size_t>(hc.cells[pos]) * n;
                for (int row = 0; row < hc.n_rows; ++row) {
                    if (hc.row_tpos[row] < 0) continue;
                    const int32_t slot = hc.cslot[pos * hc.n_t + hc.row_tpos[row]];
                    if (m2l_pairs_) {
                        const int32_t slot2 = hc.row_tpos2[row] >= 0 ? hc.cslot[pos * hc.n_t + hc.row_tpos2[row]] : -1;
                        if (slot < 0 && slot2 < 0) continue;
                        const double *mp = &Mp[static_cast<size_t>(hc.cells[pos]) * m2l_npar_];
                        double a = 0.0, bsum = 0.0;
                        if (row / m2l_s1_block_ >= hc.yb0) {
                            for (int j = 0; j < m2l_npar_; ++j) {
                                const bool y_odd = (j >= m2l_s1_off_.v[1] && j < m2l_s1_off_.v[2]) || j >= m2l_s1_off_.v[3];
                                (y_odd ? bsum : a) += hc.vt_all[static_cast<size_t>(j) * hc.r_pad16 + row] * mp[j];
                            }
                        } else {
                            for (int j = 0; j < m2l_ne16_; ++j) a += hc.vt_all[static_cast<size_t>(j) * hc.r_pad16 + row] * mp[j];
                            for (int j = m2l_ne16_; j < m2l_npar_; ++j) bsum += hc.vt_all[static_cast<size_t>(j) * hc.r_pad16 + row] * mp[j];
                        }
                        if (slot >= 0) cbuf[static_cast<size_t>(slot) * 2 + hc.row_off[row]] = a + bsum;
                        if (slot2 >= 0) cbuf[static_cast<size_t>(slot2) * 2 + hc.row_off2[row]] = a - bsum;
                        continue;
                    }
                    if (slot < 0) continue;
                    double s = 0.0;
                    for (int m = 0; m < n; ++m) s += hc.vt_all[static_cast<size_t>(m) * hc.r_pad16 + row] * Mv[m];
                    cbuf[static_cast<size_t>(slot) * 2 + hc.row_off[row]] = s;
                }
            }
        }
        for (size_t lc = 0; lc < m2l_host_.size(); ++lc) {
            if (m2l_batch_of_class_[lc] != static_cast<int32_t>(b)) continue;
            const HostM2lClass &hc = m2l_host_[lc];
            for (size_t pos = 0; pos < hc.cells.size(); ++pos) {
                double *Lb = L + static_cast<size_t>(hc.cells[pos]) * n;
                const double *cc = &cbuf[static_cast<size_t>(hc.cbase[pos])];
                if (m2l_pairs2_) {
                    const int n_par = m2l_s2_plan_.n_par(), ne16 = m2l_s2_plan_.ne16(), rows = hc.k_pad - hc.kp;
                    std::vector<double> sm(static_cast<size_t>(rows)), df(static_cast<size_t>(rows));
                    for (int r = 0; r < rows; ++r) {
                        sm[static_cast<size_t>(r)] = r < hc.kp ? cc[r] + cc[hc.kp + r] : cc[hc.kp + r];
                        df[static_cast<size_t>(r)] = r < hc.kp ? cc[r] - cc[hc.kp + r] : cc[hc.kp + r];
                    }
                    for (int i = 0; i < m2l_ne_; ++i) {
                        double le = 0.0, lo = 0.0;
                        for (int r = 0; r < rows; ++r) {
                            le += hc.u_all[static_cast<size_t>(r) * n_par + i] * sm[static_cast<size_t>(r)];
                            lo += hc.u_all[static_cast<size_t>(r) * n_par + ne16 + i] * df[static_cast<size_t>(r)];
                        }
                        if (i >= m2l_no_) {
                            Lb[i] += le;
                        } else {
                            Lb[i] += le + lo;
                            Lb[m2l_rho(i)] += le - lo;
                        }
                    }
                    continue;
                }
                for (int i = 0; i < n; ++i) {
                    double s = 0.0;
                    for (int k = 0; k < hc.k_pad; ++k) s += hc.u_all[static_cast<size_t>(k) * n_pad + i] * cc[k];
                    Lb[i] += s;
                }
            }
        }
    }
    for (const HostM2lClass &hc : m2l_host_)
        for (int32_t c : hc.cells) {
            const size_t lc = static_cast<size_t>(&hc - m2l_host_.data());
            const M2lBatch &mb = m2l_batches_[static_cast<size_t>(m2l_batch_of_class_[lc])];
            const int want = mb.groups == 1 || m2l_group_ops_[lc].empty() ? mb.groups : static_cast<int>(m2l_group_ops_[lc].size());
            if (seen[c] != want) return BBFMM_BAD_ARGUMENT;
        }
    return BBFMM_OK;
}

void FmmTree::debug_m2l_pairs(std::vector<int32_t> *out) const {
    out->clear();
    const int d = d_;
    for (size_t i = 0; i < m2l_host_.size() + m2l_variants_.size(); ++i) {
        const HostM2lClass &h = i < m2l_host_.size() ? m2l_host_[i] : m2l_variants_[i - m2l_host_.size()];
        if (h.cells.empty()) continue;
        out->push_back(h.level);
        out->push_back(h.octant);
        out->push_back(i < m2l_host_.size() ? 0 : 1);
        const size_t n_at = out->size();
        out->push_back(0);
        int32_t n_entries = 0;
        for (size_t pos = 0; pos < h.src_tv.size(); ++pos) {
            const bool x_pair = h.src_pair[pos] >= 0 && h.src_kind[pos] == 1;
            if (h.src_pair[pos] == -2 && h.src_kind[pos] == 1) continue;
            out->push_back(x_pair ? 1 : 0);
            for (int a = 0; a < d; ++a) out->push_back(ops_.all_vecs[static_cast<size_t>(h.src_tv[pos]) * d + a]);
            ++n_entries;
        }
        (*out)[n_at] = n_entries;
    }
}

void FmmTree::debug_m2l_pairs_axes(std::vector<int32_t> *out) const {
    out->clear();
    const int d = d_;
    out->push_back(m2l_pairs_ ? m2l_axes_ : 0);
    out->push_back(static_cast<int32_t>(m2l_work_[0]));
    out->push_back(static_cast<int32_t>(m2l_work_[1]));
    for (size_t i = 0; i < m2l_host_.size() + m2l_variants_.size(); ++i) {
        const HostM2lClass &h = i < m2l_host_.size() ? m2l_host_[i] : m2l_variants_[i - m2l_host_.size()];
        if (h.cells.empty()) continue;
        const int n_blk = h.r_pad16 / m2l_s1_block_;
        out->push_back(h.level);
        out->push_back(h.octant);
        out->push_back(i < m2l_host_.size() ? 0 : 1);
        out->push_back(h.pad_cols);
        out->push_back(h.yb0);
        out->push_back(n_blk);
        const size_t n_at = out->size();
        out->push_back(0);
        for (int b = 0; b < n_blk; ++b) out->push_back(b >= h.yb0 ? 1 : 0);
        int32_t n_entries = 0;
        for (size_t pos = 0; pos < h.src_tv.size(); ++pos) {
            if (h.src_pair[pos] == -2) continue;
            out->push_back(h.src_pair[pos] >= 0 ? h.src_kind[pos] : 0);
            const bool rows = h.src_row1[pos] > h.src_row0[pos];
            out->push_back(rows ? h.src_row0[pos] / m2l_s1_block_ : -1);
            out->push_back(rows ? (h.src_row1[pos] - 1) / m2l_s1_block_ : -1);
            for (int a = 0; a < d; ++a) out->push_back(ops_.all_vecs[static_cast<size_t>(h.src_tv[pos]) * d + a]);
            ++n_entries;
        }
        (*out)[n_at] = n_entries;
    }
}

void FmmTree::debug_m2l_pairs_stage2(std::vector<int32_t> *out) const {
    out->clear();
    const int d = d_;
    for (const HostM2lClass &h : m2l_host_) {
        if (h.cells.empty()) continue;
        out->push_back(h.level);
        out->push_back(h.octant);
        out->push_back(0);
        const size_t n_at = out->size();
        out->push_back(0);
        int32_t n_entries = 0;
        for (size_t pos = 0; pos < h.tgt_tv.size(); ++pos) {
            if (h.tgt_pair[pos] == -2) continue;
            out->push_back(h.tgt_pair[pos] >= 0 ? 1 : 0);
            for (int a = 0; a < d; ++a) out->push_back(ops_.all_vecs[static_cast<size_t>(h.tgt_tv[pos]) * d + a]);
            ++n_entries;
        }
        (*out)[n_at] = n_entries;
    }
}

}
```

ferreus_rbf_rs_amd/csrc/fmm_tree.cpp:

```cpp
#include "fmm_tree_impl.hpp"

namespace bbfmm {

int FmmTree::fail(int code, const std::string &msg) {
    err_ = msg;
    return code;
}
int FmmTree::hip_fail(hipError_t e, const char *what) {
    err_ = std::string("HIP error: ") + hipGetErrorString(e) + " in " + what;
    return BBFMM_DEVICE_ERROR;
}

void FmmTree::arena_begin() {
    arena_active_ = true;
    arena_used_ = 0;
    arena_need_ = 0;
}
int FmmTree::arena_end() {
    arena_active_ = false;
    if (arena_need_ > arena_.n) {
        dfree(&arena_);
        CHK(dalloc(&arena_, arena_need_ + arena_need_ / 4));
    }
    return BBFMM_OK;
// ... 400 lines not shown
    CHK(dupload(&d_u_runs_, u_runs_.idx));
    CHK(dupload(&d_w_ptr_, t.w.ptr));
    CHK(dupload(&d_w_idx_, t.w.idx));
    {
        std::vector<int64_t> job_ptr(x_cells_.size() + 1, 0);
        std::vector<int32_t> job_runs;
        for (size_t j = 0; j < x_cells_.size(); ++j) {
            const int32_t c = x_cells_[j];
            for (int64_t r = x_runs_.ptr[c]; r < x_runs_.ptr[c + 1]; ++r) {
                job_runs.push_back(x_runs_.idx[2 * r]);
                job_runs.push_back(x_runs_.idx[2 * r + 1]);
            }
            job_ptr[j + 1] = static_cast<int64_t>(job_runs.size() / 2);
        }
        CHK(dupload(&d_x_cells_, x_cells_));
        CHK(dupload(&d_x_job_run_ptr_, job_ptr));
        CHK(dupload(&d_x_runs_, job_runs));
    }
    StageTimer ut;
    HIPCHK(hipStreamSynchronize(stream_));
    ut.lap("  upload: tree, run lists");
    m2l_classes_h_.resize(m2l_host_.size() + m2l_variants_.size());
    const bool compressed = ops_.compression != kCompressionNone;
    DevBuf<int32_t> d_invperm;
    CHK(dupload(&d_invperm, ops_.invperm));
    std::vector<DevBuf<double>> d_level_ops(ops_.m2l.size());
    std::vector<std::vector<int64_t>> u_off(ops_.m2l.size()), vt_off(ops_.m2l.size());
    for (size_t lv = 0; lv < ops_.m2l.size(); ++lv) {
        std::vector<double> buf;
        for (const M2lOperator &op : ops_.m2l[lv]) {
            u_off[lv].push_back(static_cast<int64_t>(buf.size()));
            buf.insert(buf.end(), op.u.begin(), op.u.end());
            vt_off[lv].push_back(static_cast<int64_t>(buf.size()));
            buf.insert(buf.end(), op.vt.begin(), op.vt.end());
        }
        if (!buf.empty()) CHK(dupload(&d_level_ops[lv], buf));
    }
    if (shared_basis_) {
        if (!compressed) return fail(BBFMM_BAD_ARGUMENT, "BBFMM_FLAG_M2L_SHARED_BASIS needs compressed M2L operators (ACA or SVD)");
        CHK(build_shared_basis(&d_level_ops));
    }
    const int m2l_len = shared_basis_ ? basis_pad_ : cheb_.n_pad;
    std::vector<DevBuf<double>> natural_tmp;
    std::vector<DevBuf<M2lAssembleTv>> assemble_tmp;
    for (size_t i = 0; i < m2l_host_.size() + m2l_variants_.size(); ++i) {
        HostM2lClass &h = i < m2l_host_.size() ? m2l_host_[i] : m2l_variants_[i - m2l_host_.size()];
        M2lClass &c = m2l_classes_h_[i];
        std::memset(&c, 0, sizeof c);
        c.n_rows = h.n_rows;
        c.r_pad16 = h.r_pad16;
        c.n_t = h.n_t;
        c.k_pad = h.k_pad;
        c.kp = h.kp;
        c.yb0 = h.yb0;
        c.n_cells = static_cast<int32_t>(h.cells.size());
        if (h.cells.empty()) continue;
        DevBuf<double> vt, ua;
        DevBuf<int32_t> rt, rt2, ro, ce, cs;
        DevBuf<int64_t> cb;
        {
            const size_t nvt = static_cast<size_t>(m2l_pairs_ ? m2l_npar_ : cheb_.n_pad) * h.r_pad16, nu = m2l_pairs2_ ? static_cast<size_t>(h.k_pad - h.kp) * m2l_s2_plan_.n_par() : static_cast<size_t>(h.k_pad) * cheb_.n_pad;
            CHK(dalloc(&vt, nvt));
            CHK(dalloc(&ua, nu));
            const auto &lops = ops_.m2l[h.level];
            std::vector<M2lAssembleTv> src_tv, tgt_tv;
            int max_rank = 0;
            for (size_t pos = 0; pos < h.src_tv.size(); ++pos) {
                if (m2l_pairs_ && h.src_pair[pos] == -2) continue;
                const int tv = h.src_tv[pos];
                const int ref = ops_.ref_lookup[tv];
                const int rank = lops[ref].rank;
                src_tv.push_back(M2lAssembleTv{ops_.perm_lookup[tv], rank, h.src_row0[pos], vt_off[h.level][ref], u_off[h.level][ref]});
            }
            for (size_t pos = 0; pos < h.tgt_tv.size(); ++pos) {
                if (m2l_pairs2_ && h.tgt_pair[pos] == -2) continue;
                const int tv = h.tgt_tv[pos];
                const int ref = ops_.ref_lookup[tv];
                const int rank = lops[ref].rank;
                max_rank = std::max(max_rank, rank);
                const int row = m2l_pairs2_ && h.tgt_pair[pos] < 0 ? h.tgt_off[pos] - h.kp : h.tgt_off[pos];
                tgt_tv.push_back(M2lAssembleTv{ops_.perm_lookup[tv], rank, row, vt_off[h.level][ref], u_off[h.level][ref]});
            }
            DevBuf<M2lAssembleTv> d_src, d_tgt;
            CHK(dupload(&d_src, src_tv));
            CHK(dupload(&d_tgt, tgt_tv));
            const M2lAssembleClass ac{d_src.p, d_tgt.p, static_cast<int32_t>(src_tv.size()), static_cast<int32_t>(tgt_tv.size()),
                                      h.r_pad16, h.k_pad, max_rank,
                                      m2l_pairs_ ? m2l_ne_ : 0, m2l_no_, m2l_ne16_, m2l_npar_, ops_.p,
                                      m2l_pairs2_ ? m2l_s2_plan_.n_par() : 0, m2l_s2_plan_.ne16(), h.k_pad - h.kp, m2l_ne_, m2l_no_,
                                      m2l_axes_, m2l_s1_off_};
            static const bool host_fill = std::getenv("BBFMM_M2L_ASSEMBLE_HOST") != nullptr;
            if (host_fill) {
                std::vector<double> hv, hu;
                fill_m2l_operator_arrays(h, &hv, &hu);
                HIPCHK(hipMemcpy(vt.p, hv.data(), hv.size() * sizeof(double), hipMemcpyHostToDevice));
                HIPCHK(hipMemcpy(ua.p, hu.data(), hu.size() * sizeof(double), hipMemcpyHostToDevice));
            } else {
                launch_m2l_assemble(ac, ops_.n, cheb_.n_pad, compressed, d_level_ops[h.level].p, d_invperm.p, vt.p, ua.p, stream_);
            }
            assemble_tmp.push_back(d_src);
            assemble_tmp.push_back(d_tgt);
            if (shared_basis_) {
                DevBuf<double> vt2, ua2;
                CHK(dalloc(&vt2, static_cast<size_t>(m2l_len) * h.r_pad16));
                CHK(dalloc(&ua2, static_cast<size_t>(h.k_pad) * m2l_len));
                const double *W = d_basis_c_[static_cast<size_t>(h.level)].p;
                launch_small_gemm(true, m2l_len, h.r_pad16, cheb_.n_pad, W, m2l_len, vt.p, h.r_pad16, vt2.p, h.r_pad16, stream_);
                launch_small_gemm(false, h.k_pad, m2l_len, cheb_.n_pad, ua.p, cheb_.n_pad, W, m2l_len, ua2.p, m2l_len, stream_);
                natural_tmp.push_back(vt);
                natural_tmp.push_back(ua);
                vt = vt2;
                ua = ua2;
            }
        }
        CHK(dupload(&rt, h.row_dst));
        CHK(dupload(&rt2, h.row_dst2));
        CHK(dupload(&ro, h.blk_t0));
        CHK(dupload(&ce, h.cells));
        CHK(dalloc(&cs, h.cslot.size()));
        if (!h.cslot.empty()) HIPCHK(hipMemcpy(cs.p, h.cslot.data(), h.cslot.size() * sizeof(int32_t), hipMemcpyHostToDevice));
        CHK(dupload(&cb, h.cbase));
        c.vt_all = vt.p;
        c.u_all = ua.p;
        c.row_dst = rt.p;
        c.row_dst2 = rt2.p;
        c.blk_t0 = ro.p;
        c.cells = ce.p;
        c.cslot = cs.p;
        c.cbase = cb.p;
        decltype(h.cslot)().swap(h.cslot);
    }
    HIPCHK(hipStreamSynchronize(stream_));
    HIPCHK(hipGetLastError());
    for (auto &b : assemble_tmp) dfree(&b);
    for (auto &b : natural_tmp) dfree(&b);
    for (auto &b : d_level_ops) dfree(&b);
    dfree(&d_invperm);
    ut.lap("  upload: M2L operators, tables");
    CHK(dupload(&d_m2l_classes_, m2l_classes_h_));
    CHK(dupload(&d_m2l_tiles_, m2l_tiles_h_));
    CHK(dupload(&d_m2l_tiles1_, m2l_tiles1_h_));
    CHK(dupload(&d_tile_idx1_, m2l_tile_idx1_h_));
    CHK(dupload(&d_m2l_tiles2_, m2l_tiles2_h_));
// ... 310 lines not shown
            launch_m2l_parity2(d_M_.p, cheb_.n_pad, d_Mp_.p, m2l_npar_, m2l_s1_off_, ops_.p, ops_.n / (ops_.p * ops_.p), static_cast<int64_t>(k) * C, stream_);
        else
            launch_m2l_parity(d_M_.p, cheb_.n_pad, d_Mp_.p, m2l_npar_, m2l_ne16_, m2l_ne_, m2l_no_, ops_.p, static_cast<int64_t>(k) * C, stream_);
        phase_end(kPhM2L1);
    }
    double *l_out = shared_basis_ ? d_Lc_.p : s2_pairs ? d_Lp_.p : d_L_.p;
    if (shared_basis_) {
        phase_begin();
        launch_m2l_basis(d_basis_classes_.p, d_basis_tiles_c_.p, n_basis_tiles_, cheb_.n_pad, basis_pad_, k, C, d_M_.p, d_Mc_.p, stream_);
        HIPCHK(hipMemsetAsync(d_Lc_.p, 0, static_cast<size_t>(k) * C * basis_pad_ * sizeof(double), stream_));
        phase_end(kPhM2L1);
    }
    const int nb = static_cast<int>(m2l_batches_.size());
    for (int k0 = 0; k0 < k; k0 += m2l_rhs_chunk_) {
        const int kb = std::min(m2l_rhs_chunk_, k - k0);
        const double *m_chunk = m_in + static_cast<size_t>(k0) * C * s1_len;
        double *l_chunk = s2_pairs ? d_Lp_.p : l_out + static_cast<size_t>(k0) * C * m2l_len;
        if (s2_pairs) HIPCHK(hipMemsetAsync(d_Lp_.p, 0, static_cast<size_t>(kb) * C * lp_len * sizeof(double), stream_));
        for (int b = 0; b < nb; ++b) {
            const M2lBatch &mb = m2l_batches_[static_cast<size_t>(b)];
            const int t1_first = dp ? dp->batch_t1[4 * b] : mb.t1_first, t1_count = dp ? dp->batch_t1[4 * b + 1] : mb.t1_count;
            const int t2_first = dp ? dp->batch_t2[2 * b] : mb.t2_first, t2_count = dp ? dp->batch_t2[2 * b + 1] : mb.t2_count;
            if (t2_count == 0) continue;
            phase_begin();
            if (nb > 1)
                launch_m2l_zero_segments(d_m2l_zero_.p + 2 * m2l_zero_ptr_[static_cast<size_t>(b)],
                                         m2l_zero_ptr_[static_cast<size_t>(b) + 1] - m2l_zero_ptr_[static_cast<size_t>(b)], kb, d_cbuf_.p,
                                         cbuf_batch_len_, stream_);
            if (dp) {
                launch_m2l_stage1(d_m2l_classes_.p, dp->d_tiles1.p + t1_first, dp->d_tile_idx.p, t1_count, s1_len, m2l_slot_t_, kb,
                                  C, m_chunk, d_cbuf_.p, cbuf_batch_len_, stream_, false, m2l_max_blocks_, s1_ne16, m2l_s_ee_, m2l_s_eo_);
                launch_m2l_stage1(d_m2l_classes_.p, dp->d_tiles1.p + dp->batch_t1[4 * b + 2], dp->d_tile_idx.p, dp->batch_t1[4 * b + 3],
                                  s1_len, m2l_slot_t_, kb, C, m_chunk, d_cbuf_.p, cbuf_batch_len_, stream_, true, m2l_max_blocks_, s1_ne16, m2l_s_ee_, m2l_s_eo_);
            } else
                launch_m2l_stage1(d_m2l_classes_.p, d_m2l_tiles1_.p + t1_first, d_tile_idx1_.p, t1_count, s1_len, m2l_slot_t_, kb, C,
                                  m_chunk, d_cbuf_.p, cbuf_batch_len_, stream_, false, m2l_max_blocks_, s1_ne16, m2l_s_ee_, m2l_s_eo_);
            phase_end(kPhM2L1);
            phase_begin();
            if (s2_pairs) {
                if (!launch_m2l_stage2_pairs(d_m2l_classes_.p, dp ? dp->d_tiles2.p + t2_first : d_m2l_tiles2_.p + t2_first,
                                             dp ? dp->d_tile_idx.p : nullptr, t2_count, m2l_s2_plan_, kb, C, d_cbuf_.p, cbuf_batch_len_,
                                             dp ? dp->d_qlist.p : d_m2l_qlist_.p, l_chunk, stream_, !deterministic_, &m2l_s2_last_ksplit_))
                    return fail(BBFMM_DEVICE_ERROR, "internal: no stage-2 kernel instance for the parity-basis column plan");
            } else if (dp)
                launch_m2l_stage2(d_m2l_classes_.p, dp->d_tiles2.p + t2_first, dp->d_tile_idx.p, t2_count, m2l_len, kb, C, d_cbuf_.p,
                                  cbuf_batch_len_, dp->d_qlist.p, l_chunk, stream_, !deterministic_);
            else
                launch_m2l_stage2(d_m2l_classes_.p, d_m2l_tiles2_.p + t2_first, nullptr, t2_count, m2l_len, kb, C, d_cbuf_.p,
                                  cbuf_batch_len_, d_m2l_qlist_.p, l_chunk, stream_, !deterministic_);
            phase_end(kPhM2L2);
        }
        if (s2_pairs) {
            phase_begin();
            launch_m2l_unparity(d_Lp_.p, lp_len, m2l_s2_plan_.ne16(), d_L_.p + static_cast<size_t>(k0) * C * cheb_.n_pad, ops_.n, cheb_.n_pad,
                                m2l_ne_, m2l_no_, ops_.p, static_cast<int64_t>(kb) * C, stream_);
            phase_end(kPhM2L2);
        }
    }
    if (shared_basis_) {
        phase_begin();
        launch_m2l_basis(d_basis_classes_.p, d_basis_tiles_e_.p, n_basis_tiles_, basis_pad_, cheb_.n_pad, k, C, d_Lc_.p, d_L_.p, stream_);
        phase_end(kPhM2L2);
    }
    HIPCHK(hipGetLastError());
    (void)t;
    return BBFMM_OK;
}

int FmmTree::downward_tail(int k, const DownwardPlan *dp, const TargetSet *wx) {
    const HostTree &t = tree_;
    const int64_t C = t.n_cells();
    phase_begin();
    if (t.adaptive && wx) {
        launch_wx_sym(kernel_, cheb_, wx->n_wx_jobs, wx->wx_tb.p, wx->wx_te.p, wx->wx_range.p, wx->n_wxl_jobs, wx->wxl_tb.p, wx->wxl_te.p,
                      wx->wxl_range.p, d_w_idx_.p, d_centers_.p,
                      d_lengths_.p, src_ptr_, d_w_sorted_.p, t.n_points, k, d_M_.p, d_L_.p, C * cheb_.n_pad, wx->out.p,
                      static_cast<int64_t>(wx->m), wx->sym_off, static_cast<int>(wx->m), stream_);
    } else if (t.adaptive) {
        if (dp)
            launch_p2l(kernel_, cheb_, dp->n_x_jobs, dp->d_x_cells.p, dp->d_x_ptr.p, dp->d_x_runs.p, d_centers_.p,
                       d_lengths_.p, src_ptr_, d_w_sorted_.p, t.n_points, k, C, d_L_.p, stream_);
        else
            launch_p2l(kernel_, cheb_, static_cast<int>(x_cells_.size()), d_x_cells_.p, d_x_job_run_ptr_.p,
                       d_x_runs_.p, d_centers_.p, d_lengths_.p, src_ptr_, d_w_sorted_.p, t.n_points, k, C, d_L_.p,
                       stream_);
    }
    phase_end(kPhP2L);
    phase_begin();
    for (int level = 2; level <= t.depth; ++level) {
        const int rc = launch_l2l(cheb_, k, C, d_level_cells_[level].p, static_cast<int>(level_cells_[level].size()), d_parent_.p,
                                  d_octant_.p, dp ? dp->d_active.p : d_active_.p, d_L_.p, stream_);
        if (rc != 0) return hip_fail(static_cast<hipError_t>(rc), "L2L: dynamic LDS attribute");
    }
    phase_end(kPhL2L);
    HIPCHK(hipGetLastError());
    have_locals_ = dp == nullptr;
    return BBFMM_OK;
}

hipError_t FmmTree::columns_to_host(double *dst, int64_t ld, const double *d_src, int64_t m, int ncols) {
    if (m <= 0 || ncols <= 0) return hipSuccess;
    if (ld == m) return hipMemcpyAsync(dst, d_src, static_cast<size_t>(m) * ncols * sizeof(double), hipMemcpyDeviceToHost, stream_);
    for (int j = 0; j < ncols; ++j) {
        const hipError_t e = hipMemcpyAsync(dst + static_cast<size_t>(j) * ld, d_src + static_cast<size_t>(j) * m,
                                            static_cast<size_t>(m) * sizeof(double), hipMemcpyDeviceToHost, stream_);
        if (e != hipSuccess) return e;
    }
    return hipSuccess;
// ... 682 lines not shown
```

ferreus_rbf_rs_amd/csrc/fmm_tree.hpp:

```cpp
#pragma once
#include <hip/hip_runtime.h>

#include <cstdint>
#include <string>
#include <memory>
#include <vector>

#include "device.hpp"
#include "targets.hpp"
#include "ferreus_bbfmm_hip.h"
#include "kernels.hpp"
#include "operators.hpp"
#include "parallel.hpp"
#include "tree.hpp"
#include "tree_device.hpp"

namespace bbfmm {

enum Phase {
    kPhGather = 0, kPhP2M, kPhM2M, kPhM2L1, kPhM2L2, kPhP2L, kPhL2L, kPhP2P, kPhM2P, kPhL2P, kPhScatter,
    kNumPhases
};
static_assert(kNumPhases == BBFMM_N_PHASES, "phase table");

template <class T> struct DevBuf {
    T *p = nullptr;
    size_t n = 0;
    bool borrowed = false;
};

struct HostM2lClass {
    int level = 0, octant = 0;
    int n_rows = 0, r_pad16 = 16, n_t = 0, k_pad = 16;
    std::vector<double> vt_all, u_all;
    std::vector<int> src_tv, tgt_tv, tgt_off;
    std::vector<int32_t> row_tpos, row_off, row_dst, blk_t0, cells;
    std::vector<int32_t, DefaultInitAllocator<int32_t>> cslot;
    std::vector<int32_t> src_row0, src_row1;
    std::vector<int32_t> row_tpos2, row_off2, row_dst2;
    std::vector<int32_t> src_pair;
    std::vector<int8_t> src_kind;
    int yb0 = 0;
    int pad_cols = 0;
    int kp = 0;
    std::vector<int32_t> tgt_pair;
    std::vector<int64_t> cbase;
};

struct M2lBatch {
    int level_lo = 0, level_hi = 0;
    int groups = 1, group = 0;
    int64_t len = 0;
    int32_t t1_first = 0, t1_count = 0;
    int32_t t2_first = 0, t2_count = 0;
};

struct TargetSet {
    int64_t m = 0;
    DevBuf<double> xyz[3];
    const double *xyz_ptr[3] = {nullptr, nullptr, nullptr};
    DevBuf<int32_t> perm;
    DevBuf<int32_t> job_cell, tgt_begin, tgt_end;
    int n_jobs = 0;
    DevBuf<int32_t> w_tgt_begin, w_tgt_end;
    DevBuf<int64_t> w_begin, w_end;
    int n_w_jobs = 0;
    DevBuf<double> out, grad;
    bool sym = false;
    int32_t sym_off = 0;
    int n_sym_jobs = 0;
    DevBuf<int32_t> sym_tb, sym_te;
    DevBuf<int64_t> sym_ptr;
    DevBuf<int32_t> sym_runs;
    int n_syml_jobs = 0;
    DevBuf<int32_t> syml_tb, syml_te;
    DevBuf<int64_t> syml_ptr;
    int n_symw_jobs = 0;
    DevBuf<int32_t> symw_tb, symw_te;
    DevBuf<int64_t> symw_ptr;
    int n_wx_jobs = 0;
    DevBuf<int32_t> wx_tb, wx_te;
    DevBuf<int64_t> wx_range;
    int n_wxl_jobs = 0;
    DevBuf<int32_t> wxl_tb, wxl_te;
    DevBuf<int64_t> wxl_range;
};

struct DownwardPlan {
    std::vector<uint8_t> active;
    std::vector<M2lTileDesc> tiles2_h;
    std::vector<M2lTileDesc> tiles1_h;
    std::vector<int32_t> batch_t1, batch_t2;
    int64_t n_tiles1_blocks = 0;
    std::vector<int32_t> tile_idx_h;
    std::vector<uint16_t> qlist_h;
    int n_x_jobs = 0;
    bool restrict_upward = false;
    int coarse_level = 0;
// ... 55 lines not shown
    int64_t partition_coarse_count() const;
    int matvec_partition_upward(const double *d_w, int64_t ldw, int k, double *d_coarse, hipStream_t comm_stream, bool near_field = true);
    int partition_subset_finish(const double *d_coarse, const int64_t *idx, int64_t n_idx, double *h_out, hipStream_t comm_stream);
    int matvec_partition_finish(const double *d_coarse, double *d_out, int64_t ldo, bool sync, hipStream_t comm_stream);
    int matvec_partition_finish_sorted(const double *d_coarse, double *d_seg, int64_t ld, hipStream_t comm_stream);
    int partition_scatter(const double *d_all, int first_part, int n_parts, int64_t m_max, int k, double *d_out, int64_t ldo);
    int matvec_partition_finish_host(const double *d_coarse, double *h_seg, int64_t ld, hipStream_t comm_stream);
    const std::vector<int64_t> &partition_bounds() const { return part_bounds_; }
    int register_subset(const int64_t *idx, int64_t n_idx, int *id_out);
    int matvec_subset_device(int id, const double *d_w, double *d_y, bool sync);
    int set_partition(int rank, int world);

    const HostTree &tree() const { return tree_; }
    const Operators &ops() const { return ops_; }
    const PodDoubles &source_points() const { return pts_; }
    int order() const { return order_; }
    const char *last_error() const { return err_.c_str(); }
    hipStream_t stream() const { return stream_; }
    bool host_only() const { return host_only_; }
    bool deterministic() const { return deterministic_; }
    bool leaves_ready() const { return nrhs_ == 1 && have_locals_; }
    void bind_device() const {
        if (device_ >= 0) (void)hipSetDevice(device_);
    }
    int device() const { return device_; }
    bool tree_built_on_device() const { return tree_built_on_device_; }
    bool last_evaluate_at_sources() const { return last_eval_at_sources_; }
    int last_evaluate_path() const { return last_eval_at_sources_ ? 1 : (last_eval_rows_of_sources_ ? 2 : 0); }
    bool targets_are_rows_of_sources(const double *x, int64_t m, int64_t ldx, std::vector<int64_t> *rows);
    bool targets_are_sources(const double *x, int64_t m, int64_t ldx) const;
    void stats(bbfmm_tree_stats *out) const;
    void set_profiling(bool on) { profiling_ = on; }
    const double *phase_ms() { collect_phase_times(); return phase_ms_; }
    const int64_t *phase_count() { collect_phase_times(); return phase_count_; }
    void reset_phase_ms() {
        collect_phase_times();
        for (double &v : phase_ms_) v = 0.0;
        for (int64_t &v : phase_count_) v = 0;
    }
    const std::vector<int64_t> &partition_rows() const { return part_rows_; }
    bool partitioned() const { return part_world_ > 1; }
    int partition_rank() const { return part_rank_; }
    const std::vector<HostM2lClass> &m2l_host() const { return m2l_host_; }
    void m2l_variant_stats(int64_t *n_variants, int64_t *n_cells) const {
        *n_variants = static_cast<int64_t>(m2l_variants_.size());
        *n_cells = 0;
        for (const HostM2lClass &v : m2l_variants_) *n_cells += static_cast<int64_t>(v.cells.size());
    }
    void debug_m2l_pairs(std::vector<int32_t> *out) const;
    bool m2l_pairs() const { return m2l_pairs_; }
    void debug_m2l_pairs_axes(std::vector<int32_t> *out) const;
    void debug_m2l_pairs_stage2(std::vector<int32_t> *out) const;
    bool m2l_pairs_stage2() const { return m2l_pairs2_; }
    int debug_m2l_s2_last_ksplit() const { return m2l_s2_last_ksplit_; }
    int debug_apply_m2l_tables_host(const double *M, double *L) const;
    int debug_get_coefficients(char which, int k, double *out);
    int debug_partition_upward_counts(int64_t *counts_out, uint8_t *reads_out, int64_t *info_out) const;

  private:
    int fail(int code, const std::string &msg);
    int hip_fail(hipError_t e, const char *what);
    int upload();
    int build_m2l_tables();
    void fill_m2l_operator_arrays(const HostM2lClass &hc, std::vector<double> *vt_all,
                                  std::vector<double> *u_all) const;
    void fill_m2l_operator_arrays(const HostM2lClass &hc, double *vt_all, double *u_all) const;
    int ensure_rhs_capacity(int k);
    int upward(int k, const DownwardPlan *dp = nullptr);
    int downward(int k, const DownwardPlan *dp = nullptr, const TargetSet *wx = nullptr);
    int downward_m2l(int k, const DownwardPlan *dp);
    int downward_tail(int k, const DownwardPlan *dp, const TargetSet *wx);
    int leaf_pass(const TargetSet &ts, int k, bool with_grads, bool fixed_plan = false);
    int leaf_pass_near(const TargetSet &ts, int k, bool with_grads, hipStream_t st, int parts, bool wx_done = false,
                       bool fixed_plan = false);
    int leaf_pass_far(const TargetSet &ts, int k, bool with_grads);
    int build_target_set(const double *x, int64_t m, int64_t ldx, TargetSet *ts, int64_t *bad_point_index,
                         std::vector<int32_t> *leaves_out = nullptr);
    int build_target_set_device(const double *x, int64_t m, int64_t ldx, TargetSet *ts, int64_t *bad_point_index,
                                std::vector<int32_t> *leaves_out, const double *const *d_x = nullptr);
    int ensure_leaf_lookup();
    int build_target_set_host(const double *x, int64_t m, int64_t ldx, TargetSet *ts, int64_t *bad_point_index,
                              std::vector<int32_t> *leaves_out);
    int build_source_target_set();
    int build_sym_runs(TargetSet *ts, const std::vector<int32_t> &job_cells, int64_t pb, int64_t pe, const std::vector<uint8_t> *part_active = nullptr);
    void free_target_set(TargetSet *ts);
    hipError_t columns_to_host(double *dst, int64_t ld, const double *d_src, int64_t m, int ncols);
    int upload_weights(const double *w, int64_t rows, int k, int64_t ldw);
    void phase_begin();
    void phase_end(int ph);
    void collect_phase_times();
    hipEvent_t get_event();

    std::string err_;
    bool host_only_ = false;
    bool deterministic_ = false;
    bool tree_built_on_device_ = false;
    DevTreePoints dev_points_;
    int order_ = 0, d_ = 0;
    KernelSpec kernel_{};
    bbfmm_params params_{};
    PodDoubles pts_;
    HostTree tree_;
    Operators ops_;
    int nrhs_ = 0;
    bool have_locals_ = false;
    bool locals_requested_ = false;
    Csr u_runs_;
    Csr x_runs_;
    std::vector<int32_t> src_leaves_;
    std::vector<std::vector<int32_t>> m2m_parents_;
    std::vector<std::vector<int32_t>> level_cells_;
    std::vector<int32_t> x_cells_;
    std::vector<HostM2lClass> m2l_host_;
    std::vector<HostM2lClass> m2l_variants_;
    std::vector<M2lTileDesc> m2l_tiles1_h_;
    std::vector<int32_t> m2l_tile_idx1_h_;
    std::vector<M2lClass> m2l_classes_h_;
    std::vector<M2lTileDesc> m2l_tiles_h_;
    std::vector<uint16_t> m2l_qlist_h_;
    std::vector<M2lBatch> m2l_batches_;
    std::vector<int32_t> m2l_batch_of_class_;
    std::vector<std::vector<int32_t>> m2l_group_ops_;
    std::vector<int32_t> m2l_zero_h_;
    std::vector<int64_t> m2l_zero_ptr_;
    int64_t cbuf_batch_len_ = 0;
    int64_t cbuf_total_len_ = 0;
    int64_t m2l_budget_bytes_ = int64_t(16384) << 20;
    int m2l_rhs_chunk_ = 1;
    double m2l_flops_k1_ = 0;
    int n_cu_ = 256;
    int device_ = -1;
    std::vector<M2lTileDesc> m2l_tiles2_h_;
    int m2l_slot_t_ = 1;
    int m2l_max_blocks_ = 1;
    int m2l_s1_block_ = kM2lS1Block;
    bool m2l_pairs_ = false;
    int m2l_ne_ = 0, m2l_no_ = 0;
    int m2l_ne16_ = 0, m2l_npar_ = 0;
    std::vector<int32_t> m2l_partner_;
    int m2l_axes_ = 1;
    M2lParityOffsets m2l_s1_off_{{0, 0, 0, 0}};
    int m2l_s_ee_ = 0, m2l_s_eo_ = 0;
    int64_t m2l_work_[2] = {0, 0};
    std::vector<int32_t> m2l_partner_y_;
    std::vector<int32_t> m2l_par_node_;
    std::vector<int8_t> m2l_par_sign_;
    int m2l_rho_y(int m) const {
        const int p2 = ops_.n / (ops_.p * ops_.p);
        return m + (ops_.p - 1 - 2 * ((m / p2) % ops_.p)) * p2;
    }
    int m2l_rho(int m) const {
        const int p1 = ops_.n / ops_.p;
        return m + (ops_.p - 1 - 2 * (m / p1)) * p1;
    }
    DevBuf<double> d_Mp_;
    bool m2l_pairs2_ = false;
    M2lS2PairsPlan m2l_s2_plan_{1, 1, 1, 1};
    DevBuf<double> d_Lp_;
    int m2l_s2_last_ksplit_ = 0;
    int part_rank_ = 0, part_world_ = 1;
    std::vector<int64_t> part_rows_, part_bounds_;
    int partition_finish_core(const double *d_coarse, hipStream_t comm_stream, int *k_out);
    bool part_empty_ = false;
    DownwardPlan part_plan_;
    std::vector<std::unique_ptr<SubsetPlan>> subset_plans_;
    uint64_t subset_clock_ = 0;
    int build_downward_plan(const std::vector<int32_t> &target_leaves, DownwardPlan *dp, bool restrict_upward = false,
                            int64_t own_b = 0, int64_t own_e = 0);
    int part_pending_k_ = 0;
    bool multipoles_partial_ = false;
    void free_downward_plan(DownwardPlan *dp);
    int subset_plan(const int64_t *idx, int64_t n_idx, SubsetPlan **out);
    uint64_t subset_key(const int64_t *idx, int64_t n_idx) const;
    bool subset_plan_cached(const int64_t *idx, int64_t n_idx, uint64_t key) const;
    uint64_t last_subset_miss_ = 0;
    int fill_subset_plan(const int64_t *idx, int64_t n_idx, SubsetPlan *sp);
    std::vector<std::unique_ptr<SubsetPlan>> registered_plans_;

    hipStream_t stream_ = nullptr;
    hipEvent_t ev_pack_ = nullptr, ev_comm_ = nullptr;
    struct PendingPhase {
        int phase;
        hipEvent_t e0, e1;
    };
    std::vector<PendingPhase> pending_;
    std::vector<hipEvent_t> event_pool_;
    hipEvent_t pending_begin_ = nullptr;
    bool profiling_ = false;
    double phase_ms_[kNumPhases] = {0};
    int64_t phase_count_[kNumPhases] = {0};
    std::vector<void *> owned_;
    template <class T> int dalloc(DevBuf<T> *b, size_t n, bool zero = false);
    template <class T> int dupload(DevBuf<T> *b, const std::vector<T> &v);
    template <class T> int talloc(DevBuf<T> *b, size_t n, bool zero = false);
    template <class T> int tupload(DevBuf<T> *b, const std::vector<T> &v);
    void arena_begin();
    int arena_end();
    template <class T> void dfree(DevBuf<T> *b);

    ChebRef cheb_{};
    DevBuf<DevCheb> d_cheb_;
    DevBuf<double> d_src_[3];
    const double *src_ptr_[3] = {nullptr, nullptr, nullptr};
    DevBuf<double> d_zero_axis_;
    DevBuf<uint8_t> arena_;
    size_t arena_used_ = 0, arena_need_ = 0;
    bool arena_active_ = false;
    DevBuf<uint64_t> d_tab_keys_;
    DevBuf<int32_t> d_tab_vals_;
    DevBuf<uint8_t> d_is_leaf_;
    DevBuf<uint8_t> d_tscratch_;
    DevLeafLookup lk_;
// ... 66 lines not shown
```

ferreus_rbf_rs_amd/fmm_tree.py:

```python
from __future__ import annotations

import ctypes
import enum
from typing import Optional

import numpy as np

from . import _lib as L


class KernelType(enum.IntEnum):
    LinearRbf = 0
    ThinPlateSplineRbf = 1
    CubicRbf = 2
    Spheroidal3Rbf = 3
    Spheroidal5Rbf = 4
    Spheroidal7Rbf = 5
    Spheroidal9Rbf = 6
    Laplacian = 7
    OneOverR2 = 8
    OneOverR4 = 9
    GaussianExt = 100
    MultiquadricExt = 101

# ... 424 lines not shown

    def permutation_tables(self):
        n = self.stats().n_nodes
        nperm = ctypes.c_int32(0)
        self._raise(self._lib.bbfmm_get_permutation_tables(self._h, ctypes.byref(nperm), None, None,
                                                           None, None))
        nvec = 7 ** self.dim
        perm = np.zeros((nperm.value, n), dtype=np.int32)
        inv = np.zeros((nperm.value, n), dtype=np.int32)
        pl = np.zeros(nvec, dtype=np.int32)
        rl = np.zeros(nvec, dtype=np.int32)
        self._raise(self._lib.bbfmm_get_permutation_tables(
            self._h, ctypes.byref(nperm), perm.ctypes.data, inv.ctypes.data, pl.ctypes.data,
            rl.ctypes.data))
        return perm, inv, pl, rl

    def points_to_leaves(self, x):
        x = self._targets(x)
        m = x.shape[0]
        cells = np.zeros(max(m, 1), dtype=np.int32)
        bad = ctypes.c_int64(-1)
        rc = self._lib.bbfmm_points_to_leaves(self._h, x.ctypes.data, m, max(m, 1),
                                              cells.ctypes.data, ctypes.byref(bad))
        self._raise(rc, bad)
        return cells[:m]

    def debug_dense_m2m(self, child_index: int):
        n = self.stats().n_nodes
        out = np.zeros((n, n), order="F")
        self._raise(self._lib.bbfmm_debug_dense_m2m(self._h, child_index, out.ctypes.data))
        return out

    def debug_m2l_variants(self):
        nv, nc = ctypes.c_int64(), ctypes.c_int64()
        self._raise(self._lib.bbfmm_debug_m2l_variants(self._h, ctypes.byref(nv), ctypes.byref(nc)))
        return nv.value, nc.value

    def debug_m2l_pairs(self, stage=1):
        fn = self._lib.bbfmm_debug_m2l_pairs if stage == 1 else self._lib.bbfmm_debug_m2l_pairs_stage2
        n, on = ctypes.c_int64(), ctypes.c_int32()
        self._raise(fn(self._h, None, 0, ctypes.byref(n), ctypes.byref(on)))
        buf = np.zeros(max(n.value, 1), dtype=np.int32)
        self._raise(fn(self._h, buf.ctypes.data, n.value, ctypes.byref(n), ctypes.byref(on)))
        d, ops, i = self.dim, [], 0
        while i < n.value:
            level, octant, kind, ne = (int(v) for v in buf[i:i + 4])
            ent = buf[i + 4:i + 4 + ne * (d + 1)].reshape(ne, d + 1)
            ops.append({"level": level, "octant": octant, "kind": kind,
                        "pairs": [tuple(int(x) for x in e[1:]) for e in ent if e[0] == 1],
                        "singles": [tuple(int(x) for x in e[1:]) for e in ent if e[0] == 0]})
            i += 4 + ne * (d + 1)
        return bool(on.value), ops

    def debug_m2l_pairs_axes(self):
        fn = self._lib.bbfmm_debug_m2l_pairs_axes
        n = ctypes.c_int64()
        self._raise(fn(self._h, None, 0, ctypes.byref(n)))
        buf = np.zeros(max(n.value, 1), dtype=np.int32)
        self._raise(fn(self._h, buf.ctypes.data, n.value, ctypes.byref(n)))
        info = {"axes": int(buf[0]), "work_x": int(buf[1]), "work_xy": int(buf[2])}
        d, ops, i = self.dim, [], 3
        while i < n.value:
            level, octant, kind, pad_cols, yb0, n_blk, ne = (int(v) for v in buf[i:i + 7])
            kinds = [int(v) for v in buf[i + 7:i + 7 + n_blk]]
            ent = buf[i + 7 + n_blk:i + 7 + n_blk + ne * (d + 3)].reshape(ne, d + 3)
            by_kind = [{tuple(int(x) for x in e[3:]): (int(e[1]), int(e[2])) for e in ent if e[0] == k} for k in range(3)]
            ops.append({"level": level, "octant": octant, "kind": kind, "pad_cols": pad_cols, "yb0": yb0, "block_kinds": kinds,
                        "singles": by_kind[0], "x_pairs": by_kind[1], "y_pairs": by_kind[2]})
            i += 7 + n_blk + ne * (d + 3)
        return info, ops

    def debug_m2l_s2_last_ksplit(self) -> int:
        ks = ctypes.c_int32()
        self._raise(self._lib.bbfmm_debug_m2l_s2_last_ksplit(self._h, ctypes.byref(ks)))
        return ks.value

    def debug_get_coefficients(self, which: str, k: int) -> np.ndarray:
        s = self.stats()
        out = np.zeros((k, s.n_cells, s.n_nodes))
        self._raise(self._lib.bbfmm_debug_get_coefficients(self._h, which.encode()[0:1], k,
                                                           out.ctypes.data))
        return out

    def debug_apply_m2l_tables_host(self, M: np.ndarray) -> np.ndarray:
        M = np.ascontiguousarray(M, dtype=np.float64)
        Lc = np.zeros_like(M)
        self._raise(self._lib.bbfmm_debug_apply_m2l_tables_host(self._h, M.ctypes.data,
                                                                Lc.ctypes.data))
        return Lc


def fp64_valu_selftest():
    tf, mhz = ctypes.c_double(0), ctypes.c_double(0)
    if L.load().bbfmm_fp64_valu_selftest(ctypes.byref(tf), ctypes.byref(mhz)) != L.OK:
        raise RuntimeError("the FP64 VALU microbenchmark needs a HIP device")
    return tf.value, mhz.value


def mfma_f64_selftest():
    tf = ctypes.c_double(0)
    errs = ctypes.c_int32(-1)
    info = (ctypes.c_double * 6)()
    rc = L.load().bbfmm_mfma_f64_selftest(ctypes.byref(tf), ctypes.byref(errs), info)
    if rc != L.OK:
        raise RuntimeError("MFMA self-test needs a HIP device")
    mfma_f64_selftest.info = dict(zip(["cycles_per_mfma_lone_wave", "clock_mhz_lone_wave",
                                       "cycles_per_mfma_per_simd_busy", "clock_mhz_busy",
# ... 26 lines not shown
```

include/ferreus_bbfmm_hip.h:

```cpp
#ifndef FERREUS_BBFMM_HIP_H
#define FERREUS_BBFMM_HIP_H

#include <stdint.h>

#ifdef __cplusplus
extern "C" {
#endif

typedef enum {
    BBFMM_OK = 0,
    BBFMM_POINT_OUTSIDE_TREE = 1,
    BBFMM_KERNEL_NO_GRADIENTS = 2,
    BBFMM_BAD_ARGUMENT = 3,
    BBFMM_DEVICE_ERROR = 4,
    BBFMM_UNSUPPORTED = 5,
    BBFMM_CALLBACK_FAILED = 6
} bbfmm_status;

typedef enum {
    BBFMM_KERNEL_LINEAR_RBF = 0,
    BBFMM_KERNEL_THIN_PLATE_SPLINE_RBF = 1,
    BBFMM_KERNEL_CUBIC_RBF = 2,
    BBFMM_KERNEL_SPHEROIDAL3_RBF = 3,
    BBFMM_KERNEL_SPHEROIDAL5_RBF = 4,
// ... 238 lines not shown

typedef struct {
    int32_t d, order, n_nodes, depth;
    int64_t n_points, n_cells, n_leaves;
    int64_t n_u, n_v, n_w, n_x;
    int64_t p2p_pairs;
    int64_t p2p_tile_bytes_k1;
    double m2l_flops_k1;
    double center[3];
    double radius;
    int64_t wx_pairs;
    int64_t wx_tile_bytes_k1;
    int32_t m2l_basis_rank;
    int32_t m2l_basis_len;
    int32_t m2l_batches;
    int32_t m2l_rhs_per_pass;
    int64_t m2l_slots_bytes_per_rhs;
    int64_t m2l_intermediate_bytes;
} bbfmm_tree_stats;

int bbfmm_get_tree_stats(const bbfmm_handle *h, bbfmm_tree_stats *out);
int bbfmm_tree_built_on_device(const bbfmm_handle *h);

int bbfmm_get_cells(const bbfmm_handle *h, uint64_t *keys, uint8_t *is_leaf);
int bbfmm_get_leaf_sources(const bbfmm_handle *h, int64_t *ptr, int64_t *idx);
int bbfmm_get_list(const bbfmm_handle *h, char which, int64_t *ptr, int32_t *idx,
                   int64_t *n_entries);
int bbfmm_get_m2l_ranks(const bbfmm_handle *h, int32_t *ranks, int32_t *n_ref_out);
int bbfmm_get_m2l_operator(const bbfmm_handle *h, int32_t level, int32_t ref, double *out);
int bbfmm_get_m2l_factors(const bbfmm_handle *h, int32_t level, int32_t ref, double *u, double *vt);
int bbfmm_get_permutation_tables(const bbfmm_handle *h, int32_t *n_perm, int32_t *perm,
                                 int32_t *invperm, int32_t *perm_lookup, int32_t *ref_lookup);
int bbfmm_points_to_leaves(const bbfmm_handle *h, const double *x, int64_t m, int64_t ldx,
                           int32_t *cell_out, int64_t *bad_point_index);

#define BBFMM_N_PHASES 11
int bbfmm_set_profiling(bbfmm_handle *h, int32_t enable);
int bbfmm_get_phase_ms(bbfmm_handle *h, double *ms_out, int64_t *count_out);
int bbfmm_reset_phase_ms(bbfmm_handle *h);

int bbfmm_mfma_f64_selftest(double *tflops, int32_t *layout_errors, double *info6);
int bbfmm_fp64_valu_selftest(double *tflops, double *clock_mhz);

int bbfmm_debug_kernel_values(int32_t where, int32_t kernel_id, double base_range, double total_sill, const double *r2,
                              int64_t n, double *value_out, double *value_g_out, double *factor_out);
int bbfmm_debug_math(int32_t where, int32_t which, const double *x, int64_t n, double *out, double *out2);

int bbfmm_debug_dense_m2m(const bbfmm_handle *h, int32_t child_index, double *out);
int bbfmm_debug_apply_m2l_tables_host(const bbfmm_handle *h, const double *M, double *L);
int bbfmm_debug_m2l_variants(const bbfmm_handle *h, int64_t *n_variants, int64_t *n_cells);
int bbfmm_debug_m2l_pairs(const bbfmm_handle *h, int32_t *out, int64_t cap, int64_t *n_out, int32_t *pairs_on);
int bbfmm_debug_m2l_pairs_axes(const bbfmm_handle *h, int32_t *out, int64_t cap, int64_t *n_out);
int bbfmm_debug_m2l_pairs_stage2(const bbfmm_handle *h, int32_t *out, int64_t cap, int64_t *n_out, int32_t *pairs_on);
int bbfmm_debug_m2l_s2_last_ksplit(const bbfmm_handle *h, int32_t *ksplit);

uint64_t bbfmm_debug_morton_encode(int32_t d, const uint64_t *anchor, uint64_t level);
void bbfmm_debug_morton_decode(int32_t d, uint64_t key, uint64_t *anchor_out, uint64_t *level_out);
int32_t bbfmm_debug_morton_neighbours(int32_t d, uint64_t key, uint64_t *keys_out);
int32_t bbfmm_debug_direction_vectors(int32_t d, int32_t *out);
int bbfmm_debug_reference_vectors(const bbfmm_handle *h, int32_t *out, int32_t *n_ref_out);

int bbfmm_debug_get_coefficients(bbfmm_handle *h, char which, int32_t k, double *out);


typedef int (*bbfmm_apply_fn)(void *user, const double *x, double *y, int64_t n);
typedef void (*bbfmm_iteration_fn)(void *user, int64_t iter, double residual, double progress);

enum { BBFMM_ACCURACY_ABSOLUTE = 0, BBFMM_ACCURACY_RELATIVE = 1 };

void bbfmm_givens_rotation(double f, double g, double *c, double *s, double *r);

int bbfmm_fgmres(int64_t n, bbfmm_apply_fn a, void *a_user, const double *b, bbfmm_apply_fn m, void *m_user,
                 const double *x0, int32_t max_outer_iterations, int32_t max_inner_iterations,
                 int32_t tolerance_type, double tolerance, bbfmm_iteration_fn callback, void *cb_user,
                 double *x, int64_t *iterations, double *final_residual);

int bbfmm_schwarz_ddm_solver(int64_t n, bbfmm_apply_fn matvec, void *a_user, const double *rhs,
                             bbfmm_apply_fn m, void *m_user, int32_t max_iterations, int32_t tolerance_type,
                             double tolerance, bbfmm_iteration_fn callback, void *cb_user, double *x,
                             int64_t *iterations, double *final_residual);

typedef struct bbfmm_rbf_system {
    bbfmm_handle *tree;
    int64_t basis_size;
    const double *monomial_matrix;
    int64_t ld_monomial;
    double nugget;
} bbfmm_rbf_system;
int bbfmm_rbf_system_apply(void *user, const double *x, double *y, int64_t n);

typedef struct bbfmm_ddm bbfmm_ddm;
typedef struct bbfmm_ddm_params {
    int64_t leaf_threshold;
    double overlap_quota;
    double coarse_ratio;
    int64_t coarse_threshold;
} bbfmm_ddm_params;
void bbfmm_ddm_params_defaults(bbfmm_ddm_params *out);
void bbfmm_ddm_params_for_points(int64_t n, bbfmm_ddm_params *out);
int bbfmm_ddm_build(const double *points, int64_t n, int32_t d, int64_t ld, const bbfmm_ddm_params *params,
                    bbfmm_ddm **out);
void bbfmm_ddm_destroy(bbfmm_ddm *t);
int32_t bbfmm_ddm_num_levels(const bbfmm_ddm *t);
int64_t bbfmm_ddm_level_size(const bbfmm_ddm *t, int32_t level);
int bbfmm_ddm_level_points(const bbfmm_ddm *t, int32_t level, int64_t *out);
int64_t bbfmm_ddm_num_domains(const bbfmm_ddm *t, int32_t level);
// ... 93 lines not shown
```

Before: 31.75 matvecs/s.

## Extend M2L stage-2 parity pairing to two symmetry axes

Adds a second symmetry axis to the M2L stage-2 parity decomposition. Targets paired along a second axis share a single sum/difference of staged coefficients, so the output is split into four parity parts (ee/eo/oe/oo) via new pairs2 MFMA kernels, a plan chooser and an unparity2 kernel. The aim is fewer MFMA products per target and less operator storage. The cost is extra register use for the second B-fragment, more template instantiations, and extra indexing in the unparity step.

Result: faster. 33.16 matvecs/s, median of 6 (+4.4%).

```diff
diff --git a/ferreus_rbf_rs_amd/_lib.py b/ferreus_rbf_rs_amd/_lib.py
--- a/ferreus_rbf_rs_amd/_lib.py
+++ b/ferreus_rbf_rs_amd/_lib.py
@@ -143,6 +143,7 @@
     "bbfmm_debug_m2l_pairs": (ctypes.c_int, [c_p, c_p, c_i64, c_p, c_p]),
     "bbfmm_debug_m2l_pairs_axes": (ctypes.c_int, [c_p, c_p, c_i64, c_p]),
     "bbfmm_debug_m2l_pairs_stage2": (ctypes.c_int, [c_p, c_p, c_i64, c_p, c_p]),
+    "bbfmm_debug_m2l_pairs_axes_stage2": (ctypes.c_int, [c_p, c_p, c_i64, c_p]),
     "bbfmm_debug_m2l_s2_last_ksplit": (ctypes.c_int, [c_p, c_p]),
     "bbfmm_debug_get_coefficients": (ctypes.c_int, [c_p, ctypes.c_char, c_i32, c_p]),
     "bbfmm_debug_morton_encode": (ctypes.c_uint64, [c_i32, c_p, ctypes.c_uint64]),
diff --git a/ferreus_rbf_rs_amd/csrc/capi.cpp b/ferreus_rbf_rs_amd/csrc/capi.cpp
--- a/ferreus_rbf_rs_amd/csrc/capi.cpp
+++ b/ferreus_rbf_rs_amd/csrc/capi.cpp
@@ -1996,6 +1996,15 @@
     return BBFMM_OK;
 }
 
+int bbfmm_debug_m2l_pairs_axes_stage2(const bbfmm_handle *h, int32_t *out, int64_t cap, int64_t *n_out) {
+    if (!h || !n_out) return BBFMM_BAD_ARGUMENT;
+    std::vector<int32_t> v;
+    h->tree.debug_m2l_pairs_axes_stage2(&v);
+    *n_out = static_cast<int64_t>(v.size());
+    if (out) std::copy(v.begin(), v.begin() + std::min<int64_t>(cap, *n_out), out);
+    return BBFMM_OK;
+}
+
 int bbfmm_debug_m2l_s2_last_ksplit(const bbfmm_handle *h, int32_t *ksplit) {
     if (!h || !ksplit) return BBFMM_BAD_ARGUMENT;
     *ksplit = h->tree.debug_m2l_s2_last_ksplit();
diff --git a/ferreus_rbf_rs_amd/csrc/device.hpp b/ferreus_rbf_rs_amd/csrc/device.hpp
--- a/ferreus_rbf_rs_amd/csrc/device.hpp
+++ b/ferreus_rbf_rs_amd/csrc/device.hpp
@@ -38,6 +38,7 @@
     const double *u_all;
     int32_t k_pad;
     int32_t kp;
+    int32_t kpy;
     const int32_t *cells;
     int32_t n_cells;
     const int32_t *cslot;
@@ -97,15 +98,25 @@
                        const uint16_t *qlist, double *L, hipStream_t s, bool allow_ksplit = true);
 struct M2lS2PairsPlan {
     int ga, gb, ce, co;
+    int ya = 0, yb = 0;
     int ne16() const { return 16 * ga * ce; }
-    int n_par() const { return 16 * (ga * ce + gb * co); }
+    __host__ __device__ int n_par() const { return 16 * (ga * ce + gb * co); }
+    __host__ __device__ int col(int part, int j) const {
+        const int g = part < 2 ? ga : gb, y = part < 2 ? ya : yb, w = 16 * ((part & 1) ? g - y : y);
+        const int jj = j % w, gl = ((part & 1) ? y : 0) + jj / 16, pp = jj % 16, paired = g / 2 * 2;
+        const int local = gl < paired ? 32 * (gl / 2) + 2 * pp + (gl & 1) : 16 * paired + pp;
+        return (part < 2 ? 0 : 16 * ga * ce) + (j / w) * 16 * g + local;
+    }
 };
 M2lS2PairsPlan m2l_s2_pairs_plan(int groups_even, int groups_odd);
+M2lS2PairsPlan m2l_s2_pairs_plan2(const int groups[4]);
 bool launch_m2l_stage2_pairs(const M2lClass *classes, const M2lTileDesc *tiles, const int32_t *tile_idx, int n_tiles,
                              const M2lS2PairsPlan &plan, int K, int64_t C, const double *cbuf, int64_t cbuf_len,
                              const uint16_t *qlist, double *Lp, hipStream_t s, bool allow_ksplit = true, int *ksplit_out = nullptr);
 void launch_m2l_unparity(const double *Lp, int n_par, int ne16, double *L, int n, int n_pad, int n_e, int n_o, int p, int64_t rows,
                          hipStream_t s);
+void launch_m2l_unparity2(const double *Lp, const M2lS2PairsPlan &plan, double *L, int n, int n_pad, int p, int p2, int64_t rows,
+                          hipStream_t s);
 void launch_m2l_zero_segments(const int32_t *segs, int64_t n_segs, int K, double *cbuf, int64_t cbuf_len, hipStream_t s);
 void launch_m2l_basis(const M2lClass *classes, const M2lTileDesc *tiles, int n_tiles, int in_ld, int out_ld, int K,
                       int64_t C, const double *in, double *out, hipStream_t s);
@@ -126,6 +137,7 @@
     int32_t u_npar, u_ne16, u_rows, u_ne, u_no;
     int32_t s1_axes;
     M2lParityOffsets s1_off;
+    M2lS2PairsPlan u_plan;
 };
 void launch_m2l_assemble(const M2lAssembleClass &c, int n, int n_pad, bool compressed, const double *ops,
                          const int32_t *invperm, double *vt_all, double *u_all, hipStream_t s);
diff --git a/ferreus_rbf_rs_amd/csrc/device_m2l.hip b/ferreus_rbf_rs_amd/csrc/device_m2l.hip
--- a/ferreus_rbf_rs_amd/csrc/device_m2l.hip
+++ b/ferreus_rbf_rs_amd/csrc/device_m2l.hip
@@ -468,7 +468,7 @@
     m2l_dispatch_chunks<2>(n_pad / 16, classes, tiles, n_tiles, n_pad, z, K, C, cbuf, cbuf_len, L, 0, qlist, ksplit > 1 ? ksplit : 0, tile_idx, s);
 }
 
-template <int NG16>
+template <int NG16, int Y = NG16>
 __device__ __forceinline__ void m2l_s2_pairs_body(const M2lClass &cls, const M2lTileDesc &tile, int n_par, int g16, bool odd,
                                                   int zk, int ksplit, int64_t C, const double *__restrict__ in, int64_t in_len,
                                                   double *__restrict__ out, const uint16_t *__restrict__ qlist,
@@ -480,6 +480,7 @@
     const int nq = tile.q_count * (zk + 1) / ksplit - q_lo;
     const uint16_t *ql = qlist + tile.q_first + q_lo;
     const int kp = cls.kp, kp16 = kp >> 4;
+    const int kpy16 = Y < NG16 ? cls.kpy >> 4 : kp16;
     const double *opbase = cls.u_all + 16 * g16;
 
     constexpr int OP_CHUNKS = 2 * NG16;
@@ -526,8 +527,10 @@
             for (int h = 0; h < 2; ++h)
                 dma16(cptr[h] + 16 * q, lds0 + (unsigned)(buf * BUF + OP_DOUBLES + (2 * wave + h) * 128) * 8u);
         }
-        return q < kp16;
+        if constexpr (Y < NG16) return q < kpy16 ? 1 : q < kp16 ? 2 : 0;
+        else return q < kp16;
     };
+    using StepKind = std::conditional_t<(Y < NG16), int, bool>;
 
     double acc[4][NG16];
 #pragma unroll
@@ -539,17 +542,18 @@
     const bool wave_live = wave * 16 < tile.count;
     const int di = lane >> 4, db = (lane >> 2) & 3, dj = lane & 3;
     const double sgn = odd ? -1.0 : 1.0;
-    bool pair_cur = false;
+    StepKind pair_cur{};
     if (nq > 0) pair_cur = stage(0, 0);
     wait_dma_and_barrier();
+    auto grp = [](auto &bs, auto &bd, int g) -> auto & { return g < Y ? bs : bd; };
     for (int sidx = 0; sidx < nq; ++sidx) {
         const double *op = lds + (sidx & 1) * BUF + lane;
         const double2 *op2 = reinterpret_cast<const double2 *>(lds + (sidx & 1) * BUF) + lane;
         const double *cx = lds + (sidx & 1) * BUF + OP_DOUBLES + wave * 256 + (bk * 4 + bj) * 2;
-        bool pair_next = false;
+        StepKind pair_next{};
         if (sidx + 1 < nq) pair_next = stage(sidx + 1, (sidx + 1) & 1);
         if (wave_live) {
-            double bq[4][4];
+            double bq[4][4], bd[4][4];
 #pragma unroll
             for (int tg = 0; tg < 4; ++tg)
 #pragma unroll
@@ -558,7 +562,7 @@
                     bq[tg][2 * eh] = y.x;
                     bq[tg][2 * eh + 1] = y.y;
                 }
-            if (pair_cur) {
+            if (pair_cur == StepKind(1)) {
 #pragma unroll
                 for (int tg = 0; tg < 4; ++tg)
 #pragma unroll
@@ -568,6 +572,26 @@
                         bq[tg][2 * eh + 1] = x.y + sgn * bq[tg][2 * eh + 1];
                     }
             }
+            if constexpr (Y < NG16) {
+                if (pair_cur == 2) {
+#pragma unroll
+                    for (int tg = 0; tg < 4; ++tg)
+#pragma unroll
+                        for (int eh = 0; eh < 2; ++eh) {
+                            const double2 x = *reinterpret_cast<const double2 *>(cx + ((tg * 2 + eh) * 16) * 2);
+                            const double y0 = bq[tg][2 * eh], y1 = bq[tg][2 * eh + 1];
+                            bq[tg][2 * eh] = x.x + y0;
+                            bq[tg][2 * eh + 1] = x.y + y1;
+                            bd[tg][2 * eh] = x.x - y0;
+                            bd[tg][2 * eh + 1] = x.y - y1;
+                        }
+                } else {
+#pragma unroll
+                    for (int tg = 0; tg < 4; ++tg)
+#pragma unroll
+                        for (int e = 0; e < 4; ++e) bd[tg][e] = bq[tg][e];
+                }
+            }
 #pragma unroll
             for (int e = 0; e < 4; ++e) {
 #pragma unroll
@@ -575,15 +599,15 @@
                     const double2 a = op2[(e * NP + pr) * 64];
 #pragma unroll
                     for (int tg = 0; tg < 4; ++tg) {
-                        acc[tg][2 * pr] = __builtin_amdgcn_mfma_f64_4x4x4f64(a.x, bq[tg][e], acc[tg][2 * pr], 0, 0, 0);
-                        acc[tg][2 * pr + 1] = __builtin_amdgcn_mfma_f64_4x4x4f64(a.y, bq[tg][e], acc[tg][2 * pr + 1], 0, 0, 0);
+                        acc[tg][2 * pr] = __builtin_amdgcn_mfma_f64_4x4x4f64(a.x, grp(bq, bd, 2 * pr)[tg][e], acc[tg][2 * pr], 0, 0, 0);
+                        acc[tg][2 * pr + 1] = __builtin_amdgcn_mfma_f64_4x4x4f64(a.y, grp(bq, bd, 2 * pr + 1)[tg][e], acc[tg][2 * pr + 1], 0, 0, 0);
                     }
                 }
                 if (NS) {
                     const double a = op[4 * NP * 128 + e * 64];
 #pragma unroll
                     for (int tg = 0; tg < 4; ++tg)
-                        acc[tg][NG16 - 1] = __builtin_amdgcn_mfma_f64_4x4x4f64(a, bq[tg][e], acc[tg][NG16 - 1], 0, 0, 0);
+                        acc[tg][NG16 - 1] = __builtin_amdgcn_mfma_f64_4x4x4f64(a, grp(bq, bd, NG16 - 1)[tg][e], acc[tg][NG16 - 1], 0, 0, 0);
                 }
             }
         }
@@ -628,6 +652,20 @@
     else m2l_s2_pairs_body<GB>(cls, tile, n_par, ce * GA + (zc - ce) * GB, true, zk, ksplit, C, in, in_len, out, qlist, tile_idx, lds);
 }
 
+template <int GA, int YA, int GB, int YB>
+__global__ __launch_bounds__(512, 1) void m2l_s2_pairs2_kernel(const M2lClass *__restrict__ classes, const M2lTileDesc *__restrict__ tiles,
+                                                               int n_par, int ce, int co, int ksplit, int64_t C,
+                                                               const double *__restrict__ in, int64_t in_len, double *__restrict__ out,
+                                                               const uint16_t *__restrict__ qlist, const int32_t *__restrict__ tile_idx) {
+    extern __shared__ double lds[];
+    const M2lTileDesc tile = tiles[blockIdx.x];
+    const M2lClass cls = classes[tile.level_class];
+    const int zcols = ce + co;
+    const int zk = (int)blockIdx.z / zcols, zc = (int)blockIdx.z - zk * zcols;
+    if (zc < ce) m2l_s2_pairs_body<GA, YA>(cls, tile, n_par, zc * GA, false, zk, ksplit, C, in, in_len, out, qlist, tile_idx, lds);
+    else m2l_s2_pairs_body<GB, YB>(cls, tile, n_par, ce * GA + (zc - ce) * GB, true, zk, ksplit, C, in, in_len, out, qlist, tile_idx, lds);
+}
+
 #define M2L_S2_PAIR_WIDTHS(X) X(13, 10) X(13, 11) X(8, 8) X(7, 7) X(5, 4) X(4, 4) X(2, 2) X(1, 1)
 #define M2L_S2_WIDTH_ENTRY(A, B) {A, B},
 static constexpr int kM2lS2PairWidths[][2] = {M2L_S2_PAIR_WIDTHS(M2L_S2_WIDTH_ENTRY)};
@@ -647,6 +685,38 @@
     return best;
 }
 
+#define M2L_S2_PAIR2_WIDTHS(X) X(13, 7, 10, 6) X(14, 8, 11, 6) X(8, 4, 8, 4) X(5, 3, 4, 2) X(4, 2, 4, 2) X(2, 1, 2, 1)
+#define M2L_S2_WIDTH2_ENTRY(A, YA, B, YB) {A, YA, B, YB},
+static constexpr int kM2lS2Pair2Widths[][4] = {M2L_S2_PAIR2_WIDTHS(M2L_S2_WIDTH2_ENTRY)};
+#undef M2L_S2_WIDTH2_ENTRY
+
+M2lS2PairsPlan m2l_s2_pairs_plan2(const int groups[4]) {
+    M2lS2PairsPlan best{2, 2, 1, 1, 1, 1};
+    int best_cost = 1 << 30;
+    auto chunks = [](int n, int w) { return std::max(1, (n + w - 1) / w); };
+    for (const auto &w : kM2lS2Pair2Widths) {
+        const int ce = std::max(chunks(groups[0], w[1]), chunks(groups[1], w[0] - w[1]));
+        const int co = std::max(chunks(groups[2], w[3]), chunks(groups[3], w[2] - w[3]));
+        const int cost = ce * (w[0] + 2) + co * (w[2] + 2);
+        if (cost < best_cost) {
+            best_cost = cost;
+            best = M2lS2PairsPlan{w[0], w[2], ce, co, w[1], w[3]};
+        }
+    }
+    return best;
+}
+
+template <int GA, int YA, int GB, int YB>
+static void m2l_s2_pairs2_launch(const M2lClass *classes, const M2lTileDesc *tiles, const int32_t *tile_idx, int n_tiles,
+                                 const M2lS2PairsPlan &plan, int ksplit, int K, int64_t C, const double *cbuf, int64_t cbuf_len,
+                                 const uint16_t *qlist, double *Lp, hipStream_t s) {
+    const size_t lds = 2 * sizeof(double) * (size_t)(2 * (GA > GB ? GA : GB) * 128 + 4096);
+    static std::atomic<uint64_t> attr_set[4] = {{0}, {0}, {0}, {0}};
+    (void)allow_large_dynamic_lds(reinterpret_cast<const void *>(&m2l_s2_pairs2_kernel<GA, YA, GB, YB>), lds, attr_set);
+    hipLaunchKernelGGL((m2l_s2_pairs2_kernel<GA, YA, GB, YB>), dim3(n_tiles, K, (plan.ce + plan.co) * ksplit), dim3(512), lds, s, classes,
+                       tiles, plan.n_par(), plan.ce, plan.co, ksplit, C, cbuf, cbuf_len, Lp, qlist, tile_idx);
+}
+
 template <int GA, int GB>
 static void m2l_s2_pairs_launch(const M2lClass *classes, const M2lTileDesc *tiles, const int32_t *tile_idx, int n_tiles,
                                 const M2lS2PairsPlan &plan, int ksplit, int K, int64_t C, const double *cbuf, int64_t cbuf_len,
@@ -664,7 +734,18 @@
     if (n_tiles == 0) return true;
     const int ksplit = m2l_s2_ksplit(static_cast<int64_t>(n_tiles) * (plan.ce + plan.co) * K, allow_ksplit);
     if (ksplit_out) *ksplit_out = ksplit;
-#define M2L_S2_DISPATCH(A, B)                                                                                            \
+    if (plan.ya > 0) {
+#define M2L_S2_DISPATCH2(A, YA, B, YB)                                                                                   \
+    if (plan.ga == A && plan.ya == YA && plan.gb == B && plan.yb == YB) {                                                \
+        m2l_s2_pairs2_launch<A, YA, B, YB>(classes, tiles, tile_idx, n_tiles, plan, ksplit, K, C, cbuf, cbuf_len, qlist, \
+                                           Lp, s);                                                                       \
+        return true;                                                                                                     \
+    }
+        M2L_S2_PAIR2_WIDTHS(M2L_S2_DISPATCH2)
+#undef M2L_S2_DISPATCH2
+        return false;
+    }
+#define M2L_S2_DISPATCH(A, B)                                                                                           \
     if (plan.ga == A && plan.gb == B) {                                                                                  \
         m2l_s2_pairs_launch<A, B>(classes, tiles, tile_idx, n_tiles, plan, ksplit, K, C, cbuf, cbuf_len, qlist, Lp, s);  \
         return true;                                                                                                     \
@@ -699,6 +780,40 @@
     const int p1 = n_e / ((p + 1) / 2);
     hipLaunchKernelGGL(m2l_unparity_kernel, dim3(static_cast<unsigned>((rows + 3) / 4)), dim3(256), 0, s, Lp, n_par, ne16, L, n, n_pad, n_e,
                        n_o, p, p1, rows);
+}
+
+__global__ __launch_bounds__(256) void m2l_unparity2_kernel(const double *__restrict__ Lp, M2lS2PairsPlan plan, double *__restrict__ L,
+                                                            int n, int n_pad, int p, int p2, int64_t rows) {
+    const int64_t row = static_cast<int64_t>(blockIdx.x) * 4 + (threadIdx.x >> 6);
+    if (row >= rows) return;
+    const int n_par = plan.n_par();
+    const double *src = Lp + row * n_par;
+    double *dst = L + row * n_pad;
+    const int h = (p + 1) / 2, f = p / 2;
+    for (int e = threadIdx.x & 63; e < h * h * p2; e += 64) {
+        const int i0 = e / (h * p2), i1 = (e - i0 * h * p2) / p2, r = e - (i0 * h + i1) * p2;
+        const int m = (i0 * p + i1) * p2 + r;
+        const int dx = (p - 1 - 2 * i0) * p * p2, dy = (p - 1 - 2 * i1) * p2;
+        const bool cx = i0 >= f, cy = i1 >= f;
+        const int je = (i0 * h + i1) * p2 + r, jo = (i0 * f + i1) * p2 + r;
+        const double ee = src[plan.col(0, je)];
+        const double eo = cy ? 0.0 : src[plan.col(1, jo)];
+        const double oe = cx ? 0.0 : src[plan.col(2, je)];
+        const double oo = cx || cy ? 0.0 : src[plan.col(3, jo)];
+        const double a = cy ? ee : ee + eo, b = ee - eo, c = cy ? oe : oe + oo, d = oe - oo;
+        dst[m] = cx ? a : a + c;
+        if (!cx) dst[m + dx] = a - c;
+        if (!cy) dst[m + dy] = cx ? b : b + d;
+        if (!cx && !cy) dst[m + dx + dy] = b - d;
+    }
+    for (int j = n + (threadIdx.x & 63); j < n_pad; j += 64) dst[j] = 0.0;
+}
+
+void launch_m2l_unparity2(const double *Lp, const M2lS2PairsPlan &plan, double *L, int n, int n_pad, int p, int p2, int64_t rows,
+                          hipStream_t s) {
+    if (rows <= 0) return;
+    hipLaunchKernelGGL(m2l_unparity2_kernel, dim3(static_cast<unsigned>((rows + 3) / 4)), dim3(256), 0, s, Lp, plan, L, n, n_pad, p, p2,
+                       rows);
 }
 
 __global__ __launch_bounds__(256) void m2l_parity_kernel(const double *__restrict__ M, int n_pad, double *__restrict__ Mp, int n_par,
@@ -932,6 +1047,30 @@
     }
 }
 
+__global__ __launch_bounds__(256) void assemble_u_parity2_kernel(M2lAssembleClass c, int n, const double *__restrict__ ops,
+                                                                 const int32_t *__restrict__ invperm, double *__restrict__ u_all) {
+    const int p = c.p, p2 = n / (p * p), h = (p + 1) / 2, f = p / 2, n_ee = h * h * p2;
+    const M2lAssembleTv tv = c.tgt[blockIdx.y];
+    const int64_t t = static_cast<int64_t>(blockIdx.x) * 256 + threadIdx.x;
+    if (t >= static_cast<int64_t>(tv.rank) * n_ee) return;
+    const int kk = static_cast<int>(t / n_ee), e = static_cast<int>(t % n_ee);
+    const int i0 = e / (h * p2), i1 = (e - i0 * h * p2) / p2, r = e - (i0 * h + i1) * p2;
+    const int m = (i0 * p + i1) * p2 + r;
+    const int dx = (p - 1 - 2 * i0) * p * p2, dy = (p - 1 - 2 * i1) * p2;
+    const bool cx = i0 >= f, cy = i1 >= f;
+    const int32_t *inv = invperm + static_cast<int64_t>(tv.perm) * n;
+    const double *ucol = ops + tv.u_off + static_cast<int64_t>(kk) * n;
+    double *dst = u_all + static_cast<int64_t>(tv.row + kk) * c.u_npar;
+    const int je = (i0 * h + i1) * p2 + r, jo = (i0 * f + i1) * p2 + r;
+    const double v = ucol[inv[m]], vx = ucol[inv[m + dx]], vy = ucol[inv[m + dy]], vxy = ucol[inv[m + dx + dy]];
+    const double w = (cx ? 1.0 : 0.5) * (cy ? 1.0 : 0.5);
+    const double e0 = cx ? v : v + vx, e1 = cx ? vy : vy + vxy, o0 = v - vx, o1 = vy - vxy;
+    dst[c.u_plan.col(0, je)] = w * (cy ? e0 : e0 + e1);
+    if (!cy) dst[c.u_plan.col(1, jo)] = w * (e0 - e1);
+    if (!cx) dst[c.u_plan.col(2, je)] = w * (cy ? o0 : o0 + o1);
+    if (!cx && !cy) dst[c.u_plan.col(3, jo)] = w * (o0 - o1);
+}
+
 void launch_m2l_assemble(const M2lAssembleClass &c, int n, int n_pad, bool compressed, const double *ops,
                          const int32_t *invperm, double *vt_all, double *u_all, hipStream_t s) {
     (void)hipMemsetAsync(vt_all, 0, static_cast<size_t>(c.n_e > 0 ? c.n_par : n_pad) * c.r_pad16 * sizeof(double), s);
@@ -946,7 +1085,11 @@
     else if (c.n_src > 0)
         hipLaunchKernelGGL(assemble_vt_kernel, dim3(static_cast<unsigned>((static_cast<int64_t>(c.n_src) * n + 255) / 256)), dim3(256), 0, s, c, n, n_pad,
                            compressed ? 1 : 0, ops, invperm, vt_all);
-    if (c.n_tgt > 0 && c.max_rank > 0 && c.u_npar > 0)
+    if (c.n_tgt > 0 && c.max_rank > 0 && c.u_npar > 0 && c.u_plan.ya > 0) {
+        const int h = (c.p + 1) / 2, n_ee = h * h * (n / (c.p * c.p));
+        hipLaunchKernelGGL(assemble_u_parity2_kernel, dim3(static_cast<unsigned>((static_cast<int64_t>(c.max_rank) * n_ee + 255) / 256), c.n_tgt),
+                           dim3(256), 0, s, c, n, ops, invperm, u_all);
+    } else if (c.n_tgt > 0 && c.max_rank > 0 && c.u_npar > 0)
         hipLaunchKernelGGL(assemble_u_parity_kernel, dim3(static_cast<unsigned>((static_cast<int64_t>(c.max_rank) * c.u_ne + 255) / 256), c.n_tgt),
                            dim3(256), 0, s, c, n, ops, invperm, u_all);
     else if (c.n_tgt > 0 && c.max_rank > 0)
diff --git a/ferreus_rbf_rs_amd/csrc/fmm_m2l_tables.cpp b/ferreus_rbf_rs_amd/csrc/fmm_m2l_tables.cpp
--- a/ferreus_rbf_rs_amd/csrc/fmm_m2l_tables.cpp
+++ b/ferreus_rbf_rs_amd/csrc/fmm_m2l_tables.cpp
@@ -97,6 +97,20 @@
             for (int kk = 0; kk < op.rank; ++kk) {
                 double *dst = u_all + static_cast<size_t>(row0 + kk) * n_par;
                 const double *ucol = &op.u[static_cast<size_t>(kk) * n];
+                for (int k = 0; m2l_s2_axes_ == 2 && k < n_par; ++k) {
+                    const int32_t *nd = &m2l_s2_node_[static_cast<size_t>(4 * k)];
+                    const int8_t *sg = &m2l_s2_sign_[static_cast<size_t>(4 * k)];
+                    if (nd[0] < 0) continue;
+                    int cnt = 0;
+                    double half[2] = {0.0, 0.0};
+                    for (int g = 0; g < 4; ++g)
+                        if (nd[g] >= 0) {
+                            half[g >> 1] += sg[g] * ucol[inv[nd[g]]];
+                            ++cnt;
+                        }
+                    dst[k] = (half[0] + half[1]) / cnt;
+                }
+                if (m2l_s2_axes_ == 2) continue;
                 for (int i = 0; i < m2l_ne_; ++i) {
                     const double a = ucol[inv[i]], b = ucol[inv[m2l_rho(i)]];
                     if (i >= m2l_no_) {
@@ -182,7 +196,7 @@
             if (ok) m2l_partner_[static_cast<size_t>(tv)] = rt;
         }
         m2l_partner_y_.assign(static_cast<size_t>(nvec), -1);
-        for (int tv = 0; tv < nvec && m2l_pairs_; ++tv) {
+        for (int tv = 0; tv < nvec && (m2l_pairs_ || m2l_pairs2_); ++tv) {
             if (comp(tv, 1) == 0) continue;
             int rt = -1;
             for (int u = 0; u < nvec && rt < 0; ++u) {
@@ -386,13 +400,16 @@
         }
     }
     std::vector<std::vector<int32_t>> tgt_pair(ncls);
+    std::vector<std::vector<int8_t>> tgt_kind(ncls);
     for (int o = 0; o < ncls; ++o) {
         const std::vector<int> &tl = tgt_list[o];
         tgt_pair[o].assign(tl.size(), -1);
+        tgt_kind[o].assign(tl.size(), 0);
         for (size_t pos = 0; m2l_pairs2_ && pos + 1 < tl.size(); ++pos)
             if (m2l_partner_[static_cast<size_t>(tl[pos])] == tl[pos + 1] && m2l_partner_[static_cast<size_t>(tl[pos + 1])] == tl[pos]) {
                 tgt_pair[o][pos] = static_cast<int32_t>(pos + 1);
                 tgt_pair[o][pos + 1] = -2;
+                tgt_kind[o][pos] = tgt_kind[o][pos + 1] = 1;
                 ++pos;
             }
     }
@@ -407,20 +424,35 @@
 
     std::vector<int32_t> pos_in_class(t.n_cells(), -1);
     int64_t bad_pairs = 0;
-    auto slot_layout = [&](int level, std::vector<std::vector<int>> *off_tgt, std::vector<int> *k_pad, std::vector<int> *kp_out = nullptr) {
+    auto slot_layout = [&](int level, std::vector<std::vector<int>> *off_tgt, std::vector<int> *k_pad, std::vector<int> *kp_out = nullptr,
+                           std::vector<int> *kpy_out = nullptr, std::vector<int> *pad_out = nullptr) {
         const auto &lops = ops_.m2l[level];
         off_tgt->assign(ncls, {});
         k_pad->assign(ncls, 0);
         if (kp_out) kp_out->assign(ncls, 0);
+        if (kpy_out) kpy_out->assign(ncls, 0);
+        if (pad_out) pad_out->assign(ncls, 0);
         for (int o = 0; o < ncls; ++o) {
-            int lead = 0;
+            int lead = 0, lead_y = 0;
+            bool has_y = false;
             for (size_t pos = 0; pos < tgt_list[o].size(); ++pos)
-                if (tgt_pair[o][pos] >= 0) lead += round_up(lops[ops_.ref_lookup[tgt_list[o][pos]]].rank, 2);
-            const int kp = round_up(lead, 16);
+                if (tgt_pair[o][pos] >= 0) {
+                    (tgt_kind[o][pos] == 2 ? lead_y : lead) += round_up(lops[ops_.ref_lookup[tgt_list[o][pos]]].rank, 2);
+                    has_y = has_y || tgt_kind[o][pos] == 2;
+                }
+            const int kp = has_y ? round_up(round_up(lead, 16) + lead_y, 16) : round_up(lead, 16);
+            const int kpy = has_y ? round_up(lead, 16) : kp;
+            if (kpy_out) (*kpy_out)[o] = kpy;
+            if (pad_out) (*pad_out)[o] = has_y ? kpy - lead : 0;
             int off = 0, off_s = 2 * kp;
+            bool in_y = false;
             for (size_t pos = 0; pos < tgt_list[o].size(); ++pos) {
                 const int seg = round_up(lops[ops_.ref_lookup[tgt_list[o][pos]]].rank, 2);
                 if (tgt_pair[o][pos] >= 0) {
+                    if (tgt_kind[o][pos] == 2 && !in_y) {
+                        off = kpy;
+                        in_y = true;
+                    }
                     (*off_tgt)[o].push_back(off);
                 } else if (tgt_pair[o][pos] == -2) {
                     (*off_tgt)[o].push_back(kp + off);
@@ -434,6 +466,107 @@
             if (kp_out) (*kp_out)[o] = kp;
         }
     };
+    m2l_s2_axes_ = 1;
+    m2l_s2_work_[0] = m2l_s2_work_[1] = 0;
+    m2l_s2_node_.clear();
+    m2l_s2_sign_.clear();
+    m2l_s2_part_.clear();
+    if (m2l_pairs2_) {
+        const int p = ops_.p, p2 = n / (p * p), h = (p + 1) / 2, f = p / 2;
+        const int len[4] = {h * h * p2, h * f * p2, f * h * p2, f * f * p2};
+        int grp[4];
+        for (int i = 0; i < 4; ++i) grp[i] = std::max(1, round_up(len[i], 16) / 16);
+        const M2lS2PairsPlan plan2 = m2l_s2_pairs_plan2(grp);
+        std::vector<std::vector<int>> list2(ncls);
+        std::vector<std::vector<int32_t>> pair2(ncls);
+        std::vector<std::vector<int8_t>> kind2(ncls);
+        for (int o = 0; o < ncls; ++o) {
+            const std::vector<int> &tl = tgt_list[o];
+            std::vector<int> where(static_cast<size_t>(nvec), -1), xs, ys, ss;
+            for (size_t i = 0; i < tl.size(); ++i) where[static_cast<size_t>(tl[i])] = static_cast<int>(i);
+            std::vector<uint8_t> used(tl.size(), 0);
+            for (size_t i = 0; i < tl.size(); ++i)
+                if (tgt_pair[o][i] != -1) {
+                    xs.push_back(tl[i]);
+                    used[i] = 1;
+                }
+            for (size_t i = 0; i < tl.size(); ++i) {
+                if (used[i]) continue;
+                const int tv = tl[i], rt = m2l_partner_y_[static_cast<size_t>(tv)];
+                const int j = rt >= 0 ? where[static_cast<size_t>(rt)] : -1;
+                if (j < 0 || j == static_cast<int>(i) || used[static_cast<size_t>(j)] || m2l_partner_y_[static_cast<size_t>(rt)] != tv) continue;
+                const bool lead = comp(tv, 1) > 0;
+                ys.push_back(lead ? tv : rt);
+                ys.push_back(lead ? rt : tv);
+                used[i] = used[static_cast<size_t>(j)] = 1;
+            }
+            for (size_t i = 0; i < tl.size(); ++i)
+                if (!used[i]) ss.push_back(tl[i]);
+            for (int part = 0; part < 3; ++part) {
+                const std::vector<int> &src = part == 0 ? xs : part == 1 ? ys : ss;
+                for (size_t i = 0; i < src.size(); ++i) {
+                    const int32_t pos = static_cast<int32_t>(list2[o].size());
+                    list2[o].push_back(src[i]);
+                    pair2[o].push_back(part == 2 ? -1 : (i & 1) ? -2 : pos + 1);
+                    kind2[o].push_back(static_cast<int8_t>(part == 2 ? 0 : part + 1));
+                }
+            }
+        }
+        auto work_of = [&](int groups) {
+            int64_t w = 0;
+            for (int level = 2; level <= t.depth; ++level) {
+                std::vector<uint8_t> has(static_cast<size_t>(ncls), 0);
+                for (int64_t c = t.level_ptr[level]; c < t.level_ptr[level + 1]; ++c) has[t.octant[c]] = 1;
+                std::vector<std::vector<int>> off_tgt;
+                std::vector<int> k_pad, kp_cls;
+                slot_layout(level, &off_tgt, &k_pad, &kp_cls);
+                for (int o = 0; o < ncls; ++o)
+                    if (has[static_cast<size_t>(o)]) w += static_cast<int64_t>((k_pad[o] - kp_cls[o]) / 16) * groups;
+            }
+            return w;
+        };
+        m2l_s2_work_[0] = work_of(m2l_s2_plan_.n_par() / 16);
+        tgt_list.swap(list2);
+        tgt_pair.swap(pair2);
+        tgt_kind.swap(kind2);
+        m2l_s2_work_[1] = work_of(plan2.n_par() / 16);
+        const char *e = std::getenv("BBFMM_M2L_S2_AXES");
+        const int want = e ? std::atoi(e) : 0;
+        if (want == 2 || (want != 1 && m2l_s2_work_[1] < m2l_s2_work_[0])) {
+            m2l_s2_axes_ = 2;
+            m2l_s2_plan_ = plan2;
+            for (int o = 0; o < ncls; ++o)
+                for (size_t i = 0; i < tgt_list[o].size(); ++i) tpos_tgt[o][tgt_list[o][i]] = static_cast<int>(i);
+            const int n_par = plan2.n_par();
+            m2l_s2_node_.assign(static_cast<size_t>(n_par) * 4, -1);
+            m2l_s2_sign_.assign(static_cast<size_t>(n_par) * 4, 0);
+            m2l_s2_part_.assign(static_cast<size_t>(n_par), -1);
+            for (int i0 = 0; i0 < h; ++i0)
+                for (int i1 = 0; i1 < h; ++i1)
+                    for (int r = 0; r < p2; ++r) {
+                        const int m = (i0 * p + i1) * p2 + r;
+                        const bool cx = i0 >= f, cy = i1 >= f;
+                        const int nodes[4] = {m, m2l_rho(m), m2l_rho_y(m), m2l_rho_y(m2l_rho(m))};
+                        const int je = (i0 * h + i1) * p2 + r, jo = (i0 * f + i1) * p2 + r;
+                        for (int part = 0; part < 4; ++part) {
+                            const bool ox = part >= 2, oy = part & 1;
+                            if ((ox && cx) || (oy && cy)) continue;
+                            const size_t k = static_cast<size_t>(plan2.col(part, oy ? jo : je));
+                            m2l_s2_part_[k] = static_cast<int8_t>(part);
+                            for (int g = 0; g < 4; ++g) {
+                                const bool gx = g & 1, gy = g & 2;
+                                if ((gx && cx) || (gy && cy)) continue;
+                                m2l_s2_node_[4 * k + g] = nodes[g];
+                                m2l_s2_sign_[4 * k + g] = static_cast<int8_t>(((gx && ox) != (gy && oy)) ? -1 : 1);
+                            }
+                        }
+                    }
+        } else {
+            tgt_list.swap(list2);
+            tgt_pair.swap(pair2);
+            tgt_kind.swap(kind2);
+        }
+    }
     std::vector<int> level_groups(static_cast<size_t>(t.depth) + 1, 1);
     std::vector<std::vector<int>> batch_of(static_cast<size_t>(t.depth) + 1, std::vector<int>(ncls, -1));
     {
@@ -495,8 +628,8 @@
         const auto &lops = ops_.m2l[level];
         auto rank_of = [&](int tv) { return lops[ops_.ref_lookup[tv]].rank; };
         std::vector<std::vector<int>> off_tgt;
-        std::vector<int> k_pad, kp_cls;
-        slot_layout(level, &off_tgt, &k_pad, &kp_cls);
+        std::vector<int> k_pad, kp_cls, kpy_cls, pad_cls;
+        slot_layout(level, &off_tgt, &k_pad, &kp_cls, &kpy_cls, &pad_cls);
         const size_t first_class = m2l_host_.size();
         auto mark_pairs = [&](const std::vector<int> &tvs, std::vector<int32_t> *src_pair) {
             return mark_pairs_at(level, m2l_axes_, tvs, src_pair, nullptr, nullptr, nullptr, nullptr);
@@ -603,6 +736,9 @@
             hc.k_pad = k_pad[o];
             hc.kp = kp_cls[o];
             hc.tgt_pair = tgt_pair[o];
+            hc.tgt_kind = tgt_kind[o];
+            hc.kpy = kpy_cls[o];
+            hc.tgt_pad = pad_cls[o];
             if (!stage1_rows(o, src_list[o], &hc)) return fail(BBFMM_BAD_ARGUMENT, "M2L slot too long for the packed row table");
             if (hc.cells.empty()) continue;
             hc.tgt_tv = tgt_list[o];
@@ -1230,11 +1366,26 @@
                         sm[static_cast<size_t>(r)] = r < hc.kp ? cc[r] + cc[hc.kp + r] : cc[hc.kp + r];
                         df[static_cast<size_t>(r)] = r < hc.kp ? cc[r] - cc[hc.kp + r] : cc[hc.kp + r];
                     }
+                    if (m2l_s2_axes_ == 2) {
+                        for (int k = 0; k < n_par; ++k) {
+                            const int part = m2l_s2_part_[static_cast<size_t>(k)];
+                            if (part < 0) continue;
+                            double acc = 0.0;
+                            for (int r = 0; r < rows; ++r) {
+                                const bool odd = r < hc.kpy ? part >= 2 : (part & 1);
+                                acc += hc.u_all[static_cast<size_t>(r) * n_par + k] * (odd ? df : sm)[static_cast<size_t>(r)];
+                            }
+                            for (int g = 0; g < 4; ++g)
+                                if (m2l_s2_node_[static_cast<size_t>(4 * k + g)] >= 0)
+                                    Lb[m2l_s2_node_[static_cast<size_t>(4 * k + g)]] += m2l_s2_sign_[static_cast<size_t>(4 * k + g)] * acc;
+                        }
+                        continue;
+                    }
                     for (int i = 0; i < m2l_ne_; ++i) {
                         double le = 0.0, lo = 0.0;
                         for (int r = 0; r < rows; ++r) {
                             le += hc.u_all[static_cast<size_t>(r) * n_par + i] * sm[static_cast<size_t>(r)];
-                            lo += hc.u_all[static_cast<size_t>(r) * n_par + ne16 + i] * df[static_cast<size_t>(r)];
+                            if (i < m2l_no_) lo += hc.u_all[static_cast<size_t>(r) * n_par + ne16 + i] * df[static_cast<size_t>(r)];
                         }
                         if (i >= m2l_no_) {
                             Lb[i] += le;
@@ -1331,8 +1482,40 @@
         out->push_back(0);
         int32_t n_entries = 0;
         for (size_t pos = 0; pos < h.tgt_tv.size(); ++pos) {
+            const bool x_member = h.tgt_kind[pos] == 1;
+            if (h.tgt_pair[pos] == -2 && x_member) continue;
+            out->push_back(h.tgt_pair[pos] >= 0 && x_member ? 1 : 0);
+            for (int a = 0; a < d; ++a) out->push_back(ops_.all_vecs[static_cast<size_t>(h.tgt_tv[pos]) * d + a]);
+            ++n_entries;
+        }
+        (*out)[n_at] = n_entries;
+    }
+}
+
+void FmmTree::debug_m2l_pairs_axes_stage2(std::vector<int32_t> *out) const {
+    out->clear();
+    const int d = d_;
+    out->push_back(m2l_pairs2_ ? m2l_s2_axes_ : 0);
+    out->push_back(static_cast<int32_t>(m2l_s2_work_[0]));
+    out->push_back(static_cast<int32_t>(m2l_s2_work_[1]));
+    for (const HostM2lClass &h : m2l_host_) {
+        if (h.cells.empty()) continue;
+        const auto &lops = ops_.m2l[h.level];
+        out->push_back(h.level);
+        out->push_back(h.octant);
+        out->push_back(h.kp);
+        out->push_back(h.kpy);
+        out->push_back(h.k_pad);
+        out->push_back(h.tgt_pad);
+        const size_t n_at = out->size();
+        out->push_back(0);
+        int32_t n_entries = 0;
+        for (size_t pos = 0; pos < h.tgt_tv.size(); ++pos) {
             if (h.tgt_pair[pos] == -2) continue;
-            out->push_back(h.tgt_pair[pos] >= 0 ? 1 : 0);
+            out->push_back(h.tgt_pair[pos] >= 0 ? h.tgt_kind[pos] : 0);
+            out->push_back(h.tgt_off[pos]);
+            out->push_back(h.tgt_pair[pos] >= 0 ? h.tgt_off[static_cast<size_t>(h.tgt_pair[pos])] : -1);
+            out->push_back(lops[ops_.ref_lookup[h.tgt_tv[pos]]].rank);
             for (int a = 0; a < d; ++a) out->push_back(ops_.all_vecs[static_cast<size_t>(h.tgt_tv[pos]) * d + a]);
             ++n_entries;
         }
diff --git a/ferreus_rbf_rs_amd/csrc/fmm_tree.cpp b/ferreus_rbf_rs_amd/csrc/fmm_tree.cpp
--- a/ferreus_rbf_rs_amd/csrc/fmm_tree.cpp
+++ b/ferreus_rbf_rs_amd/csrc/fmm_tree.cpp
@@ -476,6 +476,7 @@
         c.n_t = h.n_t;
         c.k_pad = h.k_pad;
         c.kp = h.kp;
+        c.kpy = h.kpy;
         c.yb0 = h.yb0;
         c.n_cells = static_cast<int32_t>(h.cells.size());
         if (h.cells.empty()) continue;
@@ -512,7 +513,7 @@
                                       h.r_pad16, h.k_pad, max_rank,
                                       m2l_pairs_ ? m2l_ne_ : 0, m2l_no_, m2l_ne16_, m2l_npar_, ops_.p,
                                       m2l_pairs2_ ? m2l_s2_plan_.n_par() : 0, m2l_s2_plan_.ne16(), h.k_pad - h.kp, m2l_ne_, m2l_no_,
-                                      m2l_axes_, m2l_s1_off_};
+                                      m2l_axes_, m2l_s1_off_, m2l_pairs2_ && m2l_s2_axes_ == 2 ? m2l_s2_plan_ : M2lS2PairsPlan{1, 1, 1, 1}};
             static const bool host_fill = std::getenv("BBFMM_M2L_ASSEMBLE_HOST") != nullptr;
             if (host_fill) {
                 std::vector<double> hv, hu;
@@ -929,8 +930,12 @@
         }
         if (s2_pairs) {
             phase_begin();
-            launch_m2l_unparity(d_Lp_.p, lp_len, m2l_s2_plan_.ne16(), d_L_.p + static_cast<size_t>(k0) * C * cheb_.n_pad, ops_.n, cheb_.n_pad,
-                                m2l_ne_, m2l_no_, ops_.p, static_cast<int64_t>(kb) * C, stream_);
+            if (m2l_s2_axes_ == 2)
+                launch_m2l_unparity2(d_Lp_.p, m2l_s2_plan_, d_L_.p + static_cast<size_t>(k0) * C * cheb_.n_pad, ops_.n, cheb_.n_pad, ops_.p,
+                                     ops_.n / (ops_.p * ops_.p), static_cast<int64_t>(kb) * C, stream_);
+            else
+                launch_m2l_unparity(d_Lp_.p, lp_len, m2l_s2_plan_.ne16(), d_L_.p + static_cast<size_t>(k0) * C * cheb_.n_pad, ops_.n, cheb_.n_pad,
+                                    m2l_ne_, m2l_no_, ops_.p, static_cast<int64_t>(kb) * C, stream_);
             phase_end(kPhM2L2);
         }
     }
diff --git a/ferreus_rbf_rs_amd/csrc/fmm_tree.hpp b/ferreus_rbf_rs_amd/csrc/fmm_tree.hpp
--- a/ferreus_rbf_rs_amd/csrc/fmm_tree.hpp
+++ b/ferreus_rbf_rs_amd/csrc/fmm_tree.hpp
@@ -44,6 +44,9 @@
     int pad_cols = 0;
     int kp = 0;
     std::vector<int32_t> tgt_pair;
+    std::vector<int8_t> tgt_kind;
+    int kpy = 0;
+    int tgt_pad = 0;
     std::vector<int64_t> cbase;
 };
 
@@ -205,6 +208,7 @@
     void debug_m2l_pairs_axes(std::vector<int32_t> *out) const;
     void debug_m2l_pairs_stage2(std::vector<int32_t> *out) const;
     bool m2l_pairs_stage2() const { return m2l_pairs2_; }
+    void debug_m2l_pairs_axes_stage2(std::vector<int32_t> *out) const;
     int debug_m2l_s2_last_ksplit() const { return m2l_s2_last_ksplit_; }
     int debug_apply_m2l_tables_host(const double *M, double *L) const;
     int debug_get_coefficients(char which, int k, double *out);
@@ -311,6 +315,11 @@
     M2lS2PairsPlan m2l_s2_plan_{1, 1, 1, 1};
     DevBuf<double> d_Lp_;
     int m2l_s2_last_ksplit_ = 0;
+    int m2l_s2_axes_ = 1;
+    int64_t m2l_s2_work_[2] = {0, 0};
+    std::vector<int32_t> m2l_s2_node_;
+    std::vector<int8_t> m2l_s2_sign_;
+    std::vector<int8_t> m2l_s2_part_;
     int part_rank_ = 0, part_world_ = 1;
     std::vector<int64_t> part_rows_, part_bounds_;
     int partition_finish_core(const double *d_coarse, hipStream_t comm_stream, int *k_out);
diff --git a/ferreus_rbf_rs_amd/fmm_tree.py b/ferreus_rbf_rs_amd/fmm_tree.py
--- a/ferreus_rbf_rs_amd/fmm_tree.py
+++ b/ferreus_rbf_rs_amd/fmm_tree.py
@@ -500,7 +500,24 @@
             i += 4 + ne * (d + 1)
         return bool(on.value), ops
 
-    def debug_m2l_pairs_axes(self):
+    def debug_m2l_pairs_axes(self, stage=1):
+        if stage == 2:
+            fn = self._lib.bbfmm_debug_m2l_pairs_axes_stage2
+            n = ctypes.c_int64()
+            self._raise(fn(self._h, None, 0, ctypes.byref(n)))
+            buf = np.zeros(max(n.value, 1), dtype=np.int32)
+            self._raise(fn(self._h, buf.ctypes.data, n.value, ctypes.byref(n)))
+            info = {"axes": int(buf[0]), "work_x": int(buf[1]), "work_xy": int(buf[2])}
+            d, ops, i = self.dim, [], 3
+            while i < n.value:
+                level, octant, kp, kpy, k_pad, pad, ne = (int(v) for v in buf[i:i + 7])
+                ent = buf[i + 7:i + 7 + ne * (d + 4)].reshape(ne, d + 4)
+                by_kind = [{tuple(int(x) for x in e[4:]): (int(e[1]), int(e[2]), int(e[3])) for e in ent if e[0] == k}
+                           for k in range(3)]
+                ops.append({"level": level, "octant": octant, "kp": kp, "kpy": kpy, "k_pad": k_pad, "pad": pad,
+                            "singles": by_kind[0], "x_pairs": by_kind[1], "y_pairs": by_kind[2]})
+                i += 7 + ne * (d + 4)
+            return info, ops
         fn = self._lib.bbfmm_debug_m2l_pairs_axes
         n = ctypes.c_int64()
         self._raise(fn(self._h, None, 0, ctypes.byref(n)))
diff --git a/include/ferreus_bbfmm_hip.h b/include/ferreus_bbfmm_hip.h
--- a/include/ferreus_bbfmm_hip.h
+++ b/include/ferreus_bbfmm_hip.h
@@ -314,6 +314,7 @@
 int bbfmm_debug_m2l_pairs(const bbfmm_handle *h, int32_t *out, int64_t cap, int64_t *n_out, int32_t *pairs_on);
 int bbfmm_debug_m2l_pairs_axes(const bbfmm_handle *h, int32_t *out, int64_t cap, int64_t *n_out);
 int bbfmm_debug_m2l_pairs_stage2(const bbfmm_handle *h, int32_t *out, int64_t cap, int64_t *n_out, int32_t *pairs_on);
+int bbfmm_debug_m2l_pairs_axes_stage2(const bbfmm_handle *h, int32_t *out, int64_t cap, int64_t *n_out);
 int bbfmm_debug_m2l_s2_last_ksplit(const bbfmm_handle *h, int32_t *ksplit);
 
 uint64_t bbfmm_debug_morton_encode(int32_t d, const uint64_t *anchor, uint64_t level);
```
